# clysto/tinyimgcodec

Hardware: AMD Instinct MI355X
Metric: Mpixels/s encode (DCT+quant kernel) (higher is better)
Workload: dtype f32+f64

## Files before the change

### tinyimgcodec_amd/csrc/tic_kernels.hip

```cpp
#include <hip/hip_runtime.h>
#include <hip/hip_ext.h>
#include <stdint.h>
#include <stdlib.h>
#include <string.h>
#include <type_traits>

#include "tic_hooks.h"
#include "tic_kernels.h"
#include "tic_math.h"

namespace tic {

#define TIC_DPP_QP_XOR1 0xB1
#define TIC_DPP_QP_XOR2 0x4E
#define TIC_DPP_ROW_SHL4 0x104
#define TIC_DPP_ROW_SHR4 0x114

__device__ __forceinline__ uint32_t perm_b32(uint32_t hi_src, uint32_t lo_src, uint32_t sel) {
    return __builtin_amdgcn_perm(hi_src, lo_src, sel);
}

__device__ __forceinline__ void transpose8x8_bytes(uint32_t &lo, uint32_t &hi, int i) {
    uint32_t nhi = (uint32_t)__builtin_amdgcn_update_dpp((int)hi, (int)lo, TIC_DPP_ROW_SHL4, 0xf, 0x5, false);
    uint32_t nlo = (uint32_t)__builtin_amdgcn_update_dpp((int)lo, (int)hi, TIC_DPP_ROW_SHR4, 0xf, 0xa, false);
    lo = nlo;
    hi = nhi;
    uint32_t selB = (i & 2) ? 0x03020706u : 0x05040100u;
    uint32_t plo = (uint32_t)__builtin_amdgcn_mov_dpp((int)lo, TIC_DPP_QP_XOR2, 0xf, 0xf, true);
    uint32_t phi = (uint32_t)__builtin_amdgcn_mov_dpp((int)hi, TIC_DPP_QP_XOR2, 0xf, 0xf, true);
    lo = perm_b32(plo, lo, selB);
    hi = perm_b32(phi, hi, selB);
    uint32_t selC = (i & 1) ? 0x03070105u : 0x06020400u;
    plo = (uint32_t)__builtin_amdgcn_mov_dpp((int)lo, TIC_DPP_QP_XOR1, 0xf, 0xf, true);
    phi = (uint32_t)__builtin_amdgcn_mov_dpp((int)hi, TIC_DPP_QP_XOR1, 0xf, 0xf, true);
    lo = perm_b32(plo, lo, selC);
    hi = perm_b32(phi, hi, selC);
}

__device__ __forceinline__ void transpose8x8_bytes_shfl(uint32_t &lo, uint32_t &hi, int i) {
    uint32_t row[2] = {lo, hi};
    uint32_t col_lo = 0, col_hi = 0;
    int base = (threadIdx.x & 63) & ~7;
    for (int r = 0; r < 8; r++) {
        uint32_t l = __shfl(row[0], base + r, 64), h = __shfl(row[1], base + r, 64);
        uint32_t w = (i < 4) ? l : h;
        uint32_t byte = (w >> (8 * (i & 3))) & 0xffu;
        if (r < 4)
            col_lo |= byte << (8 * r);
        else
            col_hi |= byte << (8 * (r - 4));
    }
    lo = col_lo;
    hi = col_hi;
}

__device__ __forceinline__ void wave_lds_fence() {
    __builtin_amdgcn_fence(__ATOMIC_RELEASE, "wavefront");
    __builtin_amdgcn_wave_barrier();
    __builtin_amdgcn_fence(__ATOMIC_ACQUIRE, "wavefront");
}

__device__ __forceinline__ int reflect_index(int i, int n) {
    if (i < n) return i;
    if (n >= 8) return 2 * (n - 1) - i;
    if (n == 1) return 0;
    int p = 2 * (n - 1), j = i;
    while (j >= p) j -= p;
    return j < n ? j : p - j;
}

constexpr int kWavesPerWG = 4;
constexpr int kLdsStrideDw = 68;
constexpr int kZzStrideB = 144;
constexpr int kLdsWaveBytes = 8 * kLdsStrideDw * 4;

struct Strip {
    int by, bx;
    bool valid;
    size_t oblk;
};

__device__ __forceinline__ void load_block_row(const uint8_t *__restrict__ img, int h, int w, long stride, bool aligned8,
                                               const Strip &s, int i, uint32_t &lo, uint32_t &hi) {
    lo = 0;
    hi = 0;
    if (!s.valid) return;
    int y = reflect_index(s.by * 8 + i, h);
    int x0 = s.bx * 8;
    const uint8_t *p = img + (long)y * stride + x0;
    if (aligned8 && x0 + 8 <= w) {
        uint2 v = *reinterpret_cast<const uint2 *>(p);
        lo = v.x;
        hi = v.y;
    } else {
        const uint8_t *rowp = img + (long)y * stride;
#pragma unroll
        for (int k = 0; k < 8; k++) {
            uint32_t b = rowp[reflect_index(x0 + k, w)];
            if (k < 4)
                lo |= b << (8 * k);
            else
                hi |= b << (8 * (k - 4));
        }
    }
}

__device__ __forceinline__ void transpose8x8_dwords(uint32_t *lds, int b, int i, uint32_t v[8]) {
    uint32_t *blk = lds + b * kLdsStrideDw;
#pragma unroll
    for (int u = 0; u < 8; u++) blk[u * 8 + i] = v[u];
    wave_lds_fence();
    const uint4 *rp = reinterpret_cast<const uint4 *>(blk + i * 8);
    uint4 a = rp[0], c = rp[1];
    v[0] = a.x; v[1] = a.y; v[2] = a.z; v[3] = a.w;
    v[4] = c.x; v[5] = c.y; v[6] = c.z; v[7] = c.w;
    wave_lds_fence();
}

__device__ __forceinline__ void exact_block(uint32_t colLo, uint32_t colHi, uint32_t *lds, int b, int i,
                                         const DctqConsts *__restrict__ C, int q[8]) {
    double c[8];
#pragma unroll
    for (int r = 0; r < 4; r++) {
        c[r] = (double)((int)((colLo >> (8 * r)) & 0xffu) - 128);
        c[r + 4] = (double)((int)((colHi >> (8 * r)) & 0xffu) - 128);
    }
    dct8_exact(c[0], c[1], c[2], c[3], c[4], c[5], c[6], c[7]);
    uint32_t w[8];
#pragma unroll
    for (int k = 0; k < 8; k++) w[k] = (uint32_t)__double2loint(c[k]);
    transpose8x8_dwords(lds, b, i, w);
    uint32_t wh[8];
#pragma unroll
    for (int k = 0; k < 8; k++) wh[k] = (uint32_t)__double2hiint(c[k]);
    transpose8x8_dwords(lds, b, i, wh);
#pragma unroll
    for (int k = 0; k < 8; k++) c[k] = __hiloint2double((int)wh[k], (int)w[k]);
    dct8_exact(c[0], c[1], c[2], c[3], c[4], c[5], c[6], c[7]);
    const double *div = C->div + i * 8;
#pragma unroll
    for (int v = 0; v < 8; v++) {
        q[v] = (int)rint(c[v] / div[v]);
        __builtin_amdgcn_sched_barrier(0);
    }
}

__device__ __forceinline__ void store_zigzag(uint32_t *lds, int b, int i, const uint16_t zz[8], const int q[8],
                                             int16_t *__restrict__ out, const Strip &s) {
    char *blk = reinterpret_cast<char *>(lds) + b * kZzStrideB;
#pragma unroll
    for (int v = 0; v < 8; v++) *reinterpret_cast<int16_t *>(blk + zz[v]) = (int16_t)q[v];
    wave_lds_fence();
    uint4 val = *reinterpret_cast<const uint4 *>(blk + i * 16);
    wave_lds_fence();
    if (s.valid) *reinterpret_cast<uint4 *>(out + s.oblk * 64 + i * 8) = val;
}

__device__ __forceinline__ Strip make_strip(int tile, int ntiles, int tiles_x, int bw, int b) {
    Strip s;
    int ty = tile / tiles_x;
    int tx = tile - ty * tiles_x;
    s.by = ty;
    s.bx = tx * 8 + b;
    s.valid = (tile < ntiles) && (s.bx < bw);
    s.oblk = (size_t)ty * bw + s.bx;
    return s;
}

__global__ __launch_bounds__(kWavesPerWG * 64) void dctq_exact_kernel(DctqArgs a) {
    __shared__ __attribute__((aligned(16))) uint32_t lds_all[kWavesPerWG][kLdsWaveBytes / 4];
    a.img += (long)blockIdx.y * a.frame_stride_in;
    a.out = reinterpret_cast<int16_t *>(reinterpret_cast<char *>(a.out) + (long)blockIdx.y * a.frame_stride_out);
    const int lane = threadIdx.x & 63, wave = threadIdx.x >> 6;
    const int b = lane >> 3, i = lane & 7;
    uint32_t *lds = lds_all[wave];
    int tile = blockIdx.x * kWavesPerWG + wave;
    int ntiles = a.ntiles;
    if (a.rem_mode) {
        const int bh = a.ntiles / a.tiles_x, rw = a.tiles_x - a.fast_tx;
        const int n_right = bh * rw, n_bottom = (bh - a.fast_ty) * a.fast_tx;
        ntiles = 0;
        if (tile < n_right) {
            tile = (tile / rw) * a.tiles_x + a.fast_tx + tile % rw;
            ntiles = a.ntiles;
        } else if (tile < n_right + n_bottom) {
            const int k = tile - n_right;
            tile = (a.fast_ty + k / a.fast_tx) * a.tiles_x + k % a.fast_tx;
            ntiles = a.ntiles;
        }
    }
    Strip s = make_strip(tile, ntiles, a.tiles_x, a.bw, b);
    uint32_t lo, hi;
    load_block_row(a.img, a.h, a.w, a.stride, a.aligned8, s, i, lo, hi);
    transpose8x8_bytes(lo, hi, i);
    int q[8];
    exact_block(lo, hi, lds, b, i, a.consts, q);
    const uint4 zzv = *reinterpret_cast<const uint4 *>(a.consts->zzofs + i * 8);
    uint16_t zz[8] = {(uint16_t)zzv.x, (uint16_t)(zzv.x >> 16), (uint16_t)zzv.y, (uint16_t)(zzv.y >> 16),
                      (uint16_t)zzv.z, (uint16_t)(zzv.z >> 16), (uint16_t)zzv.w, (uint16_t)(zzv.w >> 16)};
    store_zigzag(lds, b, i, zz, q, a.out, s);
}

constexpr int kTWaveBytes = kLdsWaveBytes;
constexpr int kTHalfDw = 272;
constexpr int kZzWaveBytes = 8 * kZzStrideB;
constexpr int kPxBlkBytes = 80;
constexpr int kMaxStripsPerWave = 16;
constexpr int kChunkStrips = 8;

__device__ __forceinline__ void quant_fma(float z, float mul, uint32_t &bits, float &d) {
    const float s = fmaf(z, mul, kMagic);
    bits = __float_as_uint(s);
    const float nr = kMagic - s;
    d = fmaf(z, mul, nr);
}

__device__ __forceinline__ void store16_wt_nt(void *p, const uint4 &v) {
    typedef uint32_t u32x4 __attribute__((ext_vector_type(4)));
    const u32x4 d = {v.x, v.y, v.z, v.w};
    asm volatile("global_store_dwordx4 %0, %1, off sc1 nt" : : "v"(p), "v"(d) : "memory");
}
__device__ __forceinline__ void store16_wt_nt(const void *sbase, uint32_t voff, const uint4 &v) {
    typedef uint32_t u32x4 __attribute__((ext_vector_type(4)));
    const u32x4 d = {v.x, v.y, v.z, v.w};
    asm volatile("global_store_dwordx4 %0, %1, %2 sc1 nt" : : "v"(voff), "v"(d), "s"(sbase) : "memory");
}

constexpr int kMaxStripsPerWave2 = 64;
constexpr int kBatch = 8;
constexpr int kBatchWaveBytes = kBatch * (128 + 64) + 64;

template <int CTRL>
__device__ __forceinline__ double dpp_f64(double x) {
    const int lo = __builtin_amdgcn_mov_dpp(__double2loint(x), CTRL, 0xf, 0xf, true);
    const int hi = __builtin_amdgcn_mov_dpp(__double2hiint(x), CTRL, 0xf, 0xf, true);
    return __hiloint2double(hi, lo);
}

__device__ __forceinline__ int rational_quad(const uint32_t *ldsT, int b, int i, const double *cst_rat) {
#pragma clang fp contract(off)
    const int w = i >> 2, k = i & 3;
    const uint32_t ca = (0x05010300u >> (8 * k)) & 0xffu, cb = (0x06020407u >> (8 * k)) & 0xffu;
    const uint32_t *row = ldsT + w * 128 + 4 * b;
    const float fa = __uint_as_float(row[(ca >> 2) * kTHalfDw + (ca & 3)]);
    const float fb = __uint_as_float(row[(cb >> 2) * kTHalfDw + (cb & 3)]);
    const double K = w ? (kTW3 * 0.5) : (kSq2h * 0.5);
    const double ya = (double)fa * K, yb = (double)fb * K;
    const double p = ya + yb;
    const double s2 = p + dpp_f64<TIC_DPP_QP_XOR1>(p);
    const double o = dpp_f64<TIC_DPP_QP_XOR2>(s2);
    const double E = (k & 1) ? s2 - o : s2 + o;
    const double X = E * ((k & 1) ? (kTW3 * 0.5) : (kSq2h * 0.5));
    const double div = cst_rat[2 * w + (k & 1)], rdiv = cst_rat[4 + 2 * w + (k & 1)];
    return (int)rint(div_rn(X, div, rdiv));
}

__device__ __forceinline__ int rational_slim(uint32_t rowLo, uint32_t rowHi, int i, const double *cst_rat) {
#pragma clang fp contract(off)
    uint32_t lo = perm_b32(rowHi, rowLo, 0x04030700u);
    uint32_t hi = perm_b32(rowHi, rowLo, 0x06050201u);
    transpose8x8_bytes(lo, hi, i);
    const uint32_t tot = __builtin_amdgcn_sad_u8(lo, 0u, __builtin_amdgcn_sad_u8(hi, 0u, 0u));
    const uint32_t sa = __builtin_amdgcn_sad_u8(lo & 0xff0000ffu, 0u, __builtin_amdgcn_sad_u8(hi & 0xff0000ffu, 0u, 0u));
    const int e0 = (int)tot - 1024, e4 = 2 * (int)sa - (int)tot;
    double y0 = (double)e0 * (kSq2h * 0.5);
    double y4 = (double)e4 * (kTW3 * 0.5);
    y0 = y0 + dpp_f64<TIC_DPP_QP_XOR1>(y0);
    y4 = y4 + dpp_f64<TIC_DPP_QP_XOR1>(y4);
    y0 = y0 + dpp_f64<TIC_DPP_QP_XOR2>(y0);
    y4 = y4 + dpp_f64<TIC_DPP_QP_XOR2>(y4);
    const double b0 = dpp_f64<TIC_DPP_ROW_SHL4>(y0), b4 = dpp_f64<TIC_DPP_ROW_SHL4>(y4);
    const double A = (i & 2) ? y4 : y0, B = (i & 2) ? b4 : b0;
    const double E = (i & 1) ? A - B : A + B;
    const double X = E * ((i & 1) ? (kTW3 * 0.5) : (kSq2h * 0.5));
    const double div = cst_rat[i & 3], rdiv = cst_rat[4 + (i & 3)];
    return (int)rint(div_rn(X, div, rdiv));
}
__device__ __forceinline__ unsigned long long wave_redo_block(const uint8_t *px , double *tbuf ,
                                                              const double *cosm, const double *rdiv, const uint16_t *zzofs, int16_t *img16,
                                                              int lane) {
    const int u = lane >> 3, c = lane & 7;
    typedef double d2 __attribute__((ext_vector_type(2)));
    const d2 *mu = reinterpret_cast<const d2 *>(cosm + u * 8), *mc = reinterpret_cast<const d2 *>(cosm + c * 8);
    const d2 m0 = mu[0], m1 = mu[1], m2 = mu[2], m3 = mu[3];
    double x[8];
#pragma unroll
    for (int r = 0; r < 8; r++) x[r] = (double)((int)px[r * 8 + c] - 128);
    double ta = m0.x * x[0], tb = m0.y * x[1];
    ta = fma(m1.x, x[2], ta); tb = fma(m1.y, x[3], tb);
    ta = fma(m2.x, x[4], ta); tb = fma(m2.y, x[5], tb);
    ta = fma(m3.x, x[6], ta); tb = fma(m3.y, x[7], tb);
    tbuf[u * 8 + c] = ta + tb;
    const d2 n0 = mc[0], n1 = mc[1], n2 = mc[2], n3 = mc[3];
    wave_lds_fence();
    const d2 *tu = reinterpret_cast<const d2 *>(tbuf + u * 8);
    const d2 y0 = tu[0], y1 = tu[1], y2 = tu[2], y3 = tu[3];
    double xa = n0.x * y0.x, xb = n0.y * y0.y;
    xa = fma(n1.x, y1.x, xa); xb = fma(n1.y, y1.y, xb);
    xa = fma(n2.x, y2.x, xa); xb = fma(n2.y, y2.y, xb);
    xa = fma(n3.x, y3.x, xa); xb = fma(n3.y, y3.y, xb);
    const double X = xa + xb;
    const double tq = X * rdiv[lane], rq = rint(tq);
    const bool rational = (lane & 0x1b) == 0;
    const bool decided = fabs(tq - rq) < 0.5 - 1e-9;
    if (decided && !rational) img16[zzofs[lane] >> 1] = (int16_t)(int)rq;
    const unsigned long long und = __ballot(!decided && !rational);
    wave_lds_fence();
    return und;
}

__device__ __forceinline__ uint32_t second_level_8(uint32_t colLo, uint32_t colHi, uint32_t *lds, int b, int i, const double *mul64, int q[8]) {
    double c[8];
#pragma unroll
    for (int r = 0; r < 4; r++) {
        c[r] = (double)(int)((colLo >> (8 * r)) & 0xffu);
        c[r + 4] = (double)(int)((colHi >> (8 * r)) & 0xffu);
    }
    dct8_aan(c[0], c[1], c[2], c[3], c[4], c[5], c[6], c[7]);
    c[0] -= 1024.0;
    uint32_t w[8], wh[8];
#pragma unroll
    for (int k = 0; k < 8; k++) w[k] = (uint32_t)__double2loint(c[k]);
    transpose8x8_dwords(lds, b, i, w);
#pragma unroll
    for (int k = 0; k < 8; k++) wh[k] = (uint32_t)__double2hiint(c[k]);
    transpose8x8_dwords(lds, b, i, wh);
#pragma unroll
    for (int k = 0; k < 8; k++) c[k] = __hiloint2double((int)wh[k], (int)w[k]);
    dct8_aan(c[0], c[1], c[2], c[3], c[4], c[5], c[6], c[7]);
    uint32_t und = 0;
#pragma unroll
    for (int v = 0; v < 8; v++) {
        const double t = c[v] * mul64[i * 8 + v], r = rint(t);
        q[v] = (int)r;
        if (!(fabs(t - r) < 0.5 - 1e-9)) und |= 1u << v;
    }
    return und;
}

template <bool kCols>
__global__ __launch_bounds__(kWavesPerWG * 64, 6) __attribute__((amdgpu_num_vgpr(72))) void dctq_strip_kernel(DctqArgs a) {
    __shared__ __attribute__((aligned(16))) uint32_t ldsT_all[kWavesPerWG][kTWaveBytes / 4];
    __shared__ __attribute__((aligned(16))) uint32_t ldsZ_all[kWavesPerWG][kZzWaveBytes / 4];
    __shared__ __attribute__((aligned(16))) unsigned char cst_blk[kStripBlkBytes];
    __shared__ __attribute__((aligned(16))) uint32_t bat_all[kWavesPerWG][kBatchWaveBytes / 4];
    const int lane = threadIdx.x & 63;
    const int wave = __builtin_amdgcn_readfirstlane(threadIdx.x >> 6);
    uint32_t *ldsT = ldsT_all[wave];
    char *ldsZ = reinterpret_cast<char *>(ldsZ_all[wave]);
    const uint16_t *cst_zz = reinterpret_cast<const uint16_t *>(cst_blk + kBlkZz);
    const double *cst_rat = reinterpret_cast<const double *>(cst_blk + kBlkRat);
    uint4 *bat_img = reinterpret_cast<uint4 *>(bat_all[wave]);
    uint2 *bat_pix = reinterpret_cast<uint2 *>(bat_all[wave] + kBatch * 32);
    uint32_t *bat_id = bat_all[wave] + kBatch * 48;
    const DctqConsts *__restrict__ C = a.consts;
    a.img += (long)blockIdx.z * a.frame_stride_in;
    a.out = reinterpret_cast<int16_t *>(reinterpret_cast<char *>(a.out) + (long)blockIdx.z * a.frame_stride_out);

    const int lr = lane >> 3, lb = lane & 7;
    const int b = lane >> 3, i = lane & 7;
    unsigned long long mask_exact = 0;
    uint32_t n_second = 0, n_quad = 0;
    int nE = 0;
    int t_first, n_my;
    const uint32_t st_off = (uint32_t)lane * 16u;
    {
        typedef float f32x4 __attribute__((ext_vector_type(4)));
        typedef uint32_t u32x4 __attribute__((ext_vector_type(4)));
        f32x4 m0, m1;
        f32x4 thr;
        u32x4 zzv;
        u32x4 c_fill;
        {
            constexpr int kPpw = kStripBlkPieces / kWavesPerWG;
            static_assert(kPpw * kWavesPerWG == kStripBlkPieces && kPpw <= 64, "constant block must split evenly over the waves");
            const uint32_t piece = lane < kPpw ? (uint32_t)(wave * kPpw + lane) : (uint32_t)kStripBlkPieces - 1u;
            const uint32_t fo = piece * 16u;
            asm volatile("global_load_dwordx4 v[76:79], %0, %1" : : "v"(fo), "s"(C->strip_blk) : "memory", "v76", "v77", "v78", "v79");
        }
        const uint32_t px_wr = (uint32_t)(uintptr_t)(__attribute__((address_space(3))) char *)(ldsZ + lb * kPxBlkBytes + lr * 8);
        const uint8_t *px_rd = reinterpret_cast<const uint8_t *>(ldsZ + b * kPxBlkBytes + i);
        constexpr int kHalf = kCols ? kTHalfDw : 256;
        const int p1a = kCols ? i : lr, p1b = kCols ? b : lb;
        uint32_t *twA = ldsT + (p1a >> 2) * kHalf + (p1a & 3) + 4 * p1b;
        uint32_t *twB = ldsT + (p1a >> 2) * kHalf + (p1a & 3) + 4 * (p1b ^ 4);
        const uint4 *tr = reinterpret_cast<const uint4 *>(
            __builtin_assume_aligned(ldsT + i * 32 + 4 * (b ^ (4 * ((i >> 1) & 1))), 16));
        const uint32_t ld_off = (uint32_t)(lr * (int)a.stride + lb * 8);

        uint32_t tf, t_lim;
        if (a.team_count > 0) {
            const uint32_t r = blockIdx.y;
            const uint32_t row0 = (uint32_t)((r < 8u ? a.split_lo >> (8u * r) : a.split_hi) & 0xffull);
            const uint32_t row1 = (uint32_t)((r < 7u ? a.split_lo >> (8u * r + 8u) : a.split_hi) & 0xffull);
            tf = (row0 * (uint32_t)a.team_count + blockIdx.x) * kWavesPerWG + (uint32_t)wave;
            t_lim = tf + (row1 - row0) * (uint32_t)a.tstep;
        } else if (a.round_wgs > 0) {
            const uint32_t rho = a.magic_tstep ? __umulhi(blockIdx.x, a.magic_tstep ) : blockIdx.x;
            const uint32_t wl = blockIdx.x - rho * (uint32_t)a.round_wgs;
            const uint32_t base = rho * (uint32_t)a.round_wgs * (uint32_t)a.wg_span;
            tf = base + wl * kWavesPerWG + (uint32_t)wave;
            t_lim = base + (uint32_t)a.round_wgs * (uint32_t)a.wg_span;
        } else {
            tf = blockIdx.x * (uint32_t)a.wg_stride + (uint32_t)wave;
            t_lim = blockIdx.x * (uint32_t)a.wg_stride + (uint32_t)a.wg_span;
        }
        tf = __builtin_amdgcn_readfirstlane(tf);
        const uint32_t nfast = (uint32_t)a.fast_ty * (uint32_t)a.fast_tx;
        const uint32_t t_end = t_lim < nfast ? t_lim : nfast;
        n_my = 0;
        if (tf < t_end) n_my = (a.round_wgs > 0 || a.magic_tstep == 0u) ? (int)((t_end - tf + (uint32_t)a.tstep - 1u) / (uint32_t)a.tstep)
                                                                        : (int)__umulhi(t_end - tf + (uint32_t)a.tstep - 1u, a.magic_tstep);
        if (n_my == 0) tf = 0;
        t_first = (int)tf;
        const uint32_t ty_first = a.magic_fast_tx ? __umulhi(tf, a.magic_fast_tx) : tf;
        int txp = (int)(tf - ty_first * (uint32_t)a.fast_tx);
        uint32_t in_off = ty_first * (uint32_t)(8 * a.stride) + (uint32_t)txp * 64u;
        uint32_t oblk = ty_first * (uint32_t)a.bw + (uint32_t)txp * 8u;
        uint32_t src_off = 0;
        int n_issued = 0;
        const uint8_t *img_s = a.img;
#define TIC_RSV_CLOBBER "memory", "v72", "v73", "v74", "v75", "v76", "v77", "v78", "v79"
#define TIC_LOAD(R, OB)                                                                                      \
    do {                                                                                                     \
        src_off = n_issued < n_my ? in_off : src_off;                                                        \
        OB = oblk;                                                                                           \
        asm volatile("global_load_dwordx2 v[" R "], %0, %1" : : "v"(ld_off), "s"(img_s + src_off) : TIC_RSV_CLOBBER); \
        n_issued++; txp += a.step_tx; in_off += a.in_step32; oblk += a.oblk_step;                            \
        if (__builtin_expect(txp >= a.fast_tx, 0)) { txp -= a.fast_tx; in_off += a.in_wrap32; oblk += a.oblk_wrap; } \
    } while (0)
#define TIC_TAKE_COLS(R, N) asm volatile("s_waitcnt vmcnt(" #N ")\n\tds_write_b64 %0, v[" R "]" : : "v"(px_wr) : TIC_RSV_CLOBBER)
#define TIC_TAKE_ROWS(D, R0, R1, N)                                                                          \
    asm volatile("s_waitcnt vmcnt(" #N ")\n\tv_cvt_f32_ubyte0 %0, v" #R0 "\n\tv_cvt_f32_ubyte1 %1, v" #R0 "\n\tv_cvt_f32_ubyte2 %2, v" #R0 \
                 "\n\tv_cvt_f32_ubyte3 %3, v" #R0 "\n\tv_cvt_f32_ubyte0 %4, v" #R1 "\n\tv_cvt_f32_ubyte1 %5, v" #R1                       \
                 "\n\tv_cvt_f32_ubyte2 %6, v" #R1 "\n\tv_cvt_f32_ubyte3 %7, v" #R1                                                       \
                 : "=v"(D[0]), "=v"(D[1]), "=v"(D[2]), "=v"(D[3]), "=v"(D[4]), "=v"(D[5]), "=v"(D[6]), "=v"(D[7]) : : TIC_RSV_CLOBBER)
        uint32_t ob0, ob1, ob2;
        uint32_t kstrip = 0;
        TIC_LOAD("72:73", ob0);
        TIC_LOAD("74:75", ob1);
        asm volatile("s_waitcnt vmcnt(2)\n\tv_mov_b32 %0, v76\n\tv_mov_b32 %1, v77\n\tv_mov_b32 %2, v78\n\tv_mov_b32 %3, v79"
                     : "=v"(c_fill.x), "=v"(c_fill.y), "=v"(c_fill.z), "=v"(c_fill.w) : : "memory", "v76", "v77", "v78", "v79");
        if (lane < kStripBlkPieces / kWavesPerWG) *reinterpret_cast<u32x4 *>(cst_blk + (wave * (kStripBlkPieces / kWavesPerWG) + lane) * 16) = c_fill;
        asm volatile("s_waitcnt lgkmcnt(0)\n\ts_barrier" : : : "memory");
        m0 = *reinterpret_cast<const f32x4 *>(cst_blk + (kCols ? kBlkMul : kBlkMulT) + i * 32);
        m1 = *reinterpret_cast<const f32x4 *>(cst_blk + (kCols ? kBlkMul : kBlkMulT) + i * 32 + 16);
        thr = *reinterpret_cast<const f32x4 *>(cst_blk + (kCols ? kBlkThr : kBlkThrT) + i * 16);
        zzv = *reinterpret_cast<const u32x4 *>(cst_blk + (kCols ? kBlkZz : kBlkZzT) + i * 16);
        auto zz_ptr = [&](uint32_t ofs) {
            const uint32_t c = ofs >> 4;
            return reinterpret_cast<int16_t *>(ldsZ + c * 128 + (ofs & 15) + 16 * (b ^ (kCols ? (((c >> 1) & 1) | (c & 4)) : (4 * ((c >> 1) & 1)))));
        };
        int16_t *zp0 = zz_ptr(zzv.x & 0xffff), *zp1 = zz_ptr(zzv.x >> 16), *zp2 = zz_ptr(zzv.y & 0xffff), *zp3 = zz_ptr(zzv.y >> 16);
        int16_t *zp4 = zz_ptr(zzv.z & 0xffff), *zp5 = zz_ptr(zzv.z >> 16), *zp6 = zz_ptr(zzv.w & 0xffff), *zp7 = zz_ptr(zzv.w >> 16);
        const uint4 *zr = reinterpret_cast<const uint4 *>(
            __builtin_assume_aligned(ldsZ + 16 * (i * 8 + (b ^ (kCols ? (((i >> 1) & 1) | (i & 4)) : (4 * ((i >> 1) & 1))))), 16));
        wave_lds_fence();

        int left = n_my;
        auto raw_words = [&](auto tag, uint32_t &lo, uint32_t &hi) {
            constexpr int R = decltype(tag)::value;
            static_assert(R == 72 || R == 74 || R == 76, "landing register pair");
            if constexpr (R == 72) asm volatile("v_mov_b32 %0, v72\n\tv_mov_b32 %1, v73" : "=v"(lo), "=v"(hi) : : "memory");
            else if constexpr (R == 74) asm volatile("v_mov_b32 %0, v74\n\tv_mov_b32 %1, v75" : "=v"(lo), "=v"(hi) : : "memory");
            else asm volatile("v_mov_b32 %0, v76\n\tv_mov_b32 %1, v77" : "=v"(lo), "=v"(hi) : : "memory");
        };
        auto process = [&](auto tag, const float (&pxr)[8], const uint32_t ob) {
            float d0, d1, d2, d3, d4, d5, d6, d7;
            if constexpr (kCols) {
                d0 = (float)px_rd[0]; d1 = (float)px_rd[8]; d2 = (float)px_rd[16]; d3 = (float)px_rd[24];
                d4 = (float)px_rd[32]; d5 = (float)px_rd[40]; d6 = (float)px_rd[48]; d7 = (float)px_rd[56];
            } else {
                d0 = pxr[0]; d1 = pxr[1]; d2 = pxr[2]; d3 = pxr[3]; d4 = pxr[4]; d5 = pxr[5]; d6 = pxr[6]; d7 = pxr[7];
            }
            dct8_aan(d0, d1, d2, d3, d4, d5, d6, d7);
            d0 -= 1024.0f;
            twA[0 * 32] = __float_as_uint(d0); twA[1 * 32] = __float_as_uint(d1); twB[2 * 32] = __float_as_uint(d2);
            twB[3 * 32] = __float_as_uint(d3); twA[4 * 32] = __float_as_uint(d4); twA[5 * 32] = __float_as_uint(d5);
            twB[6 * 32] = __float_as_uint(d6); twB[7 * 32] = __float_as_uint(d7);
            wave_lds_fence();
            const uint4 ra = tr[0], rb = tr[kHalf / 4];
            wave_lds_fence();
            float e0 = __uint_as_float(ra.x), e1 = __uint_as_float(ra.y), e2 = __uint_as_float(ra.z), e3 = __uint_as_float(ra.w);
            float e4 = __uint_as_float(rb.x), e5 = __uint_as_float(rb.y), e6 = __uint_as_float(rb.z), e7 = __uint_as_float(rb.w);
            dct8_aan(e0, e1, e2, e3, e4, e5, e6, e7);
            uint32_t q0, q1, q2, q3, q4, q5, q6, q7;
            float r0, r1, r2, r3, r4, r5, r6, r7;
            quant_fma(e0, m0.x, q0, r0); quant_fma(e1, m0.y, q1, r1); quant_fma(e2, m0.z, q2, r2); quant_fma(e3, m0.w, q3, r3);
            quant_fma(e4, m1.x, q4, r4); quant_fma(e5, m1.y, q5, r5); quant_fma(e6, m1.z, q6, r6); quant_fma(e7, m1.w, q7, r7);
            const float mA1 = fmaxf(fmaxf(fabsf(r1), fabsf(r2)), fabsf(r3));
            const float mA2 = fmaxf(fmaxf(fabsf(r5), fabsf(r6)), fabsf(r7));
            const float mB = fmaxf(fabsf(r0), fabsf(r4));
            const unsigned long long cA = __ballot(mA1 > thr.x) | __ballot(mA2 > thr.y);
            const unsigned long long cB = __ballot(mB > thr.z);
            *zp0 = (int16_t)q0; *zp1 = (int16_t)q1; *zp2 = (int16_t)q2; *zp3 = (int16_t)q3;
            *zp4 = (int16_t)q4; *zp5 = (int16_t)q5; *zp6 = (int16_t)q6; *zp7 = (int16_t)q7;
            const unsigned long long kRat = 0x1111111111111111ull;
            if (__builtin_expect((cB & kRat) != 0ull, 0)) {
                n_quad++;
                if constexpr (kCols) {
                    const int rq = rational_quad(ldsT, b, i, cst_rat);
                    if ((i & 2) == 0) *zz_ptr(28u * (uint32_t)(i & 1) + 20u * (uint32_t)(i >> 2) + 30u * (uint32_t)((i & 1) & (i >> 2))) = (int16_t)rq;
                } else {
                    uint32_t lo0, hi0;
                    raw_words(tag, lo0, hi0);
                    uint2 *pb = reinterpret_cast<uint2 *>(ldsT);
                    pb[lb * 8 + lr] = make_uint2(lo0, hi0);
                    wave_lds_fence();
                    const uint2 rowv = pb[lane];
                    wave_lds_fence();
                    const int rq = rational_slim(rowv.x, rowv.y, i, cst_rat);
                    if (i < 4) *zz_ptr(i == 0 ? 0u : (i == 1 ? 28u : (i == 2 ? 20u : 78u))) = (int16_t)rq;
                }
            }
            wave_lds_fence();
            const uint4 val = *zr;
            wave_lds_fence();
            const char *dst = reinterpret_cast<const char *>(a.out) + ((unsigned long long)ob << 7);
            const unsigned long long mG = cA | (cB & ~kRat);
            if (__builtin_expect(mG != 0ull, 0)) {
                const uint32_t gm = (uint32_t)__ballot(((mG >> (8u * (uint32_t)i)) & 0xffull) != 0ull) & 0xffu;
                const int nnew = __builtin_popcount(gm);
                if (nE + nnew <= kBatch && gm != 0xffu) {
                    uint32_t lo0, hi0;
                    raw_words(tag, lo0, hi0);
                    const uint32_t below = (1u << b) - 1u, lbelow = (1u << lb) - 1u;
                    const bool mine = (gm >> b) & 1u;
                    const int e = nE + __builtin_popcount(gm & below);
                    if (mine) bat_img[e * 8 + i] = val;
                    if (mine && i == 0) bat_id[e] = ob + (uint32_t)b;
                    if ((gm >> lb) & 1u) bat_pix[(nE + __builtin_popcount(gm & lbelow)) * 8 + lr] = make_uint2(lo0, hi0);
                    if (!mine) store16_wt_nt(dst, st_off, val);
                    nE += nnew;
                    n_second += (uint32_t)nnew;
                } else {
                    mask_exact |= 1ull << kstrip;
                    store16_wt_nt(dst, st_off, val);
                }
            } else
                store16_wt_nt(dst, st_off, val);
            left--;
            kstrip++;
        };
        float pxf[8] = {0.f, 0.f, 0.f, 0.f, 0.f, 0.f, 0.f, 0.f};
#define TIC_STEP(RLOAD, OBL, RTAKE, R0, R1, OBP, N)                                                          \
        TIC_LOAD(RLOAD, OBL);                                                                                \
        if constexpr (kCols) { TIC_TAKE_COLS(RTAKE, N); } else { TIC_TAKE_ROWS(pxf, R0, R1, N); }            \
        process(std::integral_constant<int, R0>(), pxf, OBP)
        do {
            if (left == 0) break;
            TIC_STEP("76:77", ob2, "72:73", 72, 73, ob0, 2);
            if (left == 0) break;
            TIC_STEP("72:73", ob0, "74:75", 74, 75, ob1, 3);
            while (left != 0) {
                TIC_STEP("74:75", ob1, "76:77", 76, 77, ob2, 4);
                if (left == 0) break;
                TIC_STEP("76:77", ob2, "72:73", 72, 73, ob0, 4);
                if (left == 0) break;
                TIC_STEP("72:73", ob0, "74:75", 74, 75, ob1, 4);
            }
        } while (0);
#undef TIC_STEP
        asm volatile("; end of the strip walk" : : : TIC_RSV_CLOBBER);
#undef TIC_LOAD
#undef TIC_TAKE_COLS
#undef TIC_TAKE_ROWS
#undef TIC_RSV_CLOBBER
    }
    if (nE != 0) {
        const double *cst_cos = reinterpret_cast<const double *>(cst_blk + kBlkCos);
        const double *cst_rdiv = reinterpret_cast<const double *>(cst_blk + kBlkRdiv);
        uint32_t m_exact = 0;
        if (nE < 3) {
            for (int ee = 0; ee < nE; ee++) {
                const unsigned long long und = wave_redo_block(reinterpret_cast<const uint8_t *>(bat_pix + ee * 8), reinterpret_cast<double *>(ldsT), cst_cos,
                                                               cst_rdiv, cst_zz, reinterpret_cast<int16_t *>(bat_img + ee * 8), lane);
                if (und != 0ull) m_exact |= 1u << ee;
            }
        } else {
            const bool have2 = b < nE;
            const int e2 = have2 ? b : 0;
            const uint2 rowv = bat_pix[e2 * 8 + i];
            uint32_t lo = rowv.x, hi = rowv.y;
            transpose8x8_bytes(lo, hi, i);
            int qs[8];
            uint32_t und = second_level_8(lo, hi, ldsT, b, i, reinterpret_cast<const double *>(cst_blk + kBlkMul64), qs);
            if ((i & 3) == 0) und &= ~0x11u;
            const uint4 zo = *reinterpret_cast<const uint4 *>(cst_zz + i * 8);
            const uint32_t zw[4] = {zo.x, zo.y, zo.z, zo.w};
            int16_t *img2 = reinterpret_cast<int16_t *>(bat_img + e2 * 8);
            if (have2) {
#pragma unroll
                for (int v = 0; v < 8; v++)
                    if (!((und >> v) & 1u) && !((i & 3) == 0 && (v & 3) == 0)) img2[((zw[v >> 1] >> (16 * (v & 1))) & 0xffffu) >> 1] = (int16_t)qs[v];
            }
            const unsigned long long um = __ballot(have2 && und != 0u);
            for (int ee = 0; ee < nE; ee++)
                if ((um >> (8 * ee)) & 0xffull) m_exact |= 1u << ee;
        }
        const bool have = b < nE;
        const int e = have ? b : 0;
        const uint32_t blk = bat_id[e];
        if (m_exact != 0u) {
            const uint2 rowv = bat_pix[e * 8 + i];
            int16_t *img16 = reinterpret_cast<int16_t *>(bat_img + e * 8);
            uint32_t lo = rowv.x, hi = rowv.y;
            transpose8x8_bytes(lo, hi, i);
            const uint4 zo = *reinterpret_cast<const uint4 *>(cst_zz + i * 8);
            const uint32_t zw[4] = {zo.x, zo.y, zo.z, zo.w};
            int qx[8];
            exact_block(lo, hi, ldsT, b, i, C, qx);
            if (have && ((m_exact >> e) & 1u)) {
#pragma unroll
                for (int v = 0; v < 8; v++) img16[((zw[v >> 1] >> (16 * (v & 1))) & 0xffffu) >> 1] = (int16_t)qx[v];
            }
        }
        wave_lds_fence();
        const uint4 val = bat_img[e * 8 + i];
        if (have) store16_wt_nt(reinterpret_cast<char *>(a.out) + ((unsigned long long)blk << 7) + (uint32_t)i * 16u, val);
    }
    if (a.fallback_count != nullptr && lane == 0) {
        if (n_second != 0) atomicAdd(a.fallback_count, (unsigned long long)n_second);
        if (n_quad != 0) atomicAdd(a.fallback_count + 1, (unsigned long long)n_quad);
        if (mask_exact != 0ull) atomicAdd(a.fallback_count + 2, (unsigned long long)__builtin_popcountll(mask_exact));
        if (nE != 0) atomicMax(a.fallback_count + 3, (unsigned long long)nE);
    }
    if (mask_exact == 0ull) return;
    asm volatile("s_waitcnt vmcnt(0)" : : : "memory");
    const uint4 zzn = *reinterpret_cast<const uint4 *>(cst_zz + i * 8);
    const uint16_t zz[8] = {(uint16_t)zzn.x, (uint16_t)(zzn.x >> 16), (uint16_t)zzn.y, (uint16_t)(zzn.y >> 16),
                            (uint16_t)zzn.z, (uint16_t)(zzn.z >> 16), (uint16_t)zzn.w, (uint16_t)(zzn.w >> 16)};
    for (unsigned long long todo = mask_exact; todo != 0ull; todo &= todo - 1ull) {
        const int k = __builtin_ctzll(todo);
        const long t = (long)t_first + (long)k * a.tstep;
        const int ty = (int)(t / a.fast_tx), tx = (int)(t - (long)ty * a.fast_tx);
        Strip s;
        s.by = ty;
        s.bx = tx * 8 + b;
        s.valid = true;
        s.oblk = (size_t)ty * a.bw + s.bx;
        uint32_t lo, hi;
        load_block_row(a.img, a.h, a.w, a.stride, true, s, i, lo, hi);
        transpose8x8_bytes(lo, hi, i);
        int q[8];
        const uint32_t und = second_level_8(lo, hi, ldsT, b, i, reinterpret_cast<const double *>(cst_blk + kBlkMul64), q);
        if (__ballot(und != 0u) != 0ull) exact_block(lo, hi, ldsT, b, i, C, q);
        store_zigzag(reinterpret_cast<uint32_t *>(ldsZ), b, i, zz, q, a.out, s);
    }
}

__global__ __launch_bounds__(kWavesPerWG * 64) void dctq_exact_wide_kernel(WideArgs a) {
    __shared__ __attribute__((aligned(16))) uint32_t lds_all[kWavesPerWG][kLdsWaveBytes / 4];
    const int lane = threadIdx.x & 63, wave = threadIdx.x >> 6;
    const int b = lane >> 3, i = lane & 7;
    uint32_t *lds = lds_all[wave];
    const int tile = blockIdx.x * kWavesPerWG + wave;
    Strip s = make_strip(tile, a.ntiles, a.tiles_x, a.bw, b);
    double c[8];
#pragma unroll
    for (int r = 0; r < 8; r++) c[r] = 0.0;
    if (s.valid) {
        const int x = reflect_index(s.bx * 8 + i, a.w);
#pragma unroll
        for (int r = 0; r < 8; r++) {
            const int y = reflect_index(s.by * 8 + r, a.h);
            c[r] = (double)a.img[(long)y * a.stride + x] - 128.0;
        }
    }
    dct8_exact(c[0], c[1], c[2], c[3], c[4], c[5], c[6], c[7]);
    uint32_t w[8], wh[8];
#pragma unroll
    for (int k = 0; k < 8; k++) w[k] = (uint32_t)__double2loint(c[k]);
    transpose8x8_dwords(lds, b, i, w);
#pragma unroll
    for (int k = 0; k < 8; k++) wh[k] = (uint32_t)__double2hiint(c[k]);
    transpose8x8_dwords(lds, b, i, wh);
#pragma unroll
    for (int k = 0; k < 8; k++) c[k] = __hiloint2double((int)wh[k], (int)w[k]);
    dct8_exact(c[0], c[1], c[2], c[3], c[4], c[5], c[6], c[7]);
    if (!s.valid) return;
    const double *div = a.consts->div + i * 8;
    const uint16_t *zz = a.consts->zzofs + i * 8;
    int32_t *ob = a.out + s.oblk * 64;
#pragma unroll
    for (int v = 0; v < 8; v++) {
        ob[zz[v] >> 1] = (int32_t)rint(c[v] / div[v]);
        __builtin_amdgcn_sched_barrier(0);
    }
}

__constant__ int kAnnScalesInt[64] = {
    16384, 22725, 21407, 19266, 16384, 12873, 8867,  4520,  22725, 31521, 29692, 26722, 22725, 17855, 12299, 6270,
    21407, 29692, 27969, 25172, 21407, 16819, 11585, 5906,  19266, 26722, 25172, 22654, 19266, 15137, 10426, 5315,
    16384, 22725, 21407, 19266, 16384, 12873, 8867,  4520,  12873, 17855, 16819, 15137, 12873, 10114, 6967,  3552,
    8867,  12299, 11585, 10426, 8867,  6967,  4799,  2446,  4520,  6270,  5906,  5315,  4520,  3552,  2446,  1247};

template <bool kWideDc, bool kMeasure = false>
__device__ __forceinline__ void idct_body(const IdctArgs &a, int wg_tile0, const SseArgs *m = nullptr) {
    __shared__ __attribute__((aligned(16))) uint32_t lds_all[kWavesPerWG][kLdsWaveBytes / 4];
    const int lane = threadIdx.x & 63, wave = threadIdx.x >> 6;
    const int b = lane >> 3, i = lane & 7;
    uint32_t *lds = lds_all[wave];
    const int tile = wg_tile0 + wave;
    const DctqConsts *__restrict__ C = a.consts;
    Strip s = make_strip(tile, a.ntiles, a.tiles_x, a.bw, b);
    if (a.first_block >= 0) {
        const long blk = a.first_block + (long)tile * 8 + b;
        s.valid = blk < a.first_block + a.nblocks_sel;
        s.by = (int)(blk / a.bw);
        s.bx = (int)(blk - (long)s.by * a.bw);
        s.oblk = (size_t)blk;
    }

    uint4 val = make_uint4(0, 0, 0, 0);
    if (s.valid) val = *reinterpret_cast<const uint4 *>(a.coeffs + s.oblk * 64 + i * 8);
    char *blk = reinterpret_cast<char *>(lds) + b * kZzStrideB;
    {
        uint32_t wv[4] = {val.x, val.y, val.z, val.w};
#pragma unroll
        for (int k = 0; k < 8; k++) {
            int nat = C->zznat[i * 8 + k];
            int16_t cv = (int16_t)((wv[k >> 1] >> (16 * (k & 1))) & 0xffffu);
            *reinterpret_cast<int16_t *>(blk + nat * 2) = cv;
        }
    }
    wave_lds_fence();
    double c[8];
#pragma unroll
    for (int u = 0; u < 8; u++) {
        int16_t cv = *reinterpret_cast<const int16_t *>(blk + (u * 8 + i) * 2);
        if (a.scaled)
            c[u] = (((double)cv / ((double)kAnnScalesInt[u * 8 + i] / 2048.0)) * a.pow2) * C->div[u * 8 + i];
        else
            c[u] = (double)cv * C->div[u * 8 + i];
    }
    if (kWideDc && i == 0 && s.valid) {
        const double dcv = (double)a.dc32[s.oblk];
        c[0] = a.scaled ? ((dcv / ((double)kAnnScalesInt[0] / 2048.0)) * a.pow2) * C->div[0] : dcv * C->div[0];
    }
    wave_lds_fence();
    idct8_exact(c[0], c[1], c[2], c[3], c[4], c[5], c[6], c[7]);
    uint32_t w[8], wh[8];
#pragma unroll
    for (int k = 0; k < 8; k++) w[k] = (uint32_t)__double2loint(c[k]);
    transpose8x8_dwords(lds, b, i, w);
#pragma unroll
    for (int k = 0; k < 8; k++) wh[k] = (uint32_t)__double2hiint(c[k]);
    transpose8x8_dwords(lds, b, i, wh);
#pragma unroll
    for (int k = 0; k < 8; k++) c[k] = __hiloint2double((int)wh[k], (int)w[k]);
    idct8_exact(c[0], c[1], c[2], c[3], c[4], c[5], c[6], c[7]);
    uint32_t px[8];
#pragma unroll
    for (int k = 0; k < 8; k++) {
        double v = c[k] + 128.0;
        v = v < 0.0 ? 0.0 : v;
        v = v > 255.0 ? 255.0 : v;
        px[k] = (uint32_t)(int)v;
    }
    if constexpr (kMeasure) {
        __shared__ uint32_t wsum[kWavesPerWG][2];
        uint32_t sq = 0, sw = 0;
        const int y = s.by * 8 + i, x0 = s.bx * 8;
        if (s.valid && y < a.h) {
            const uint8_t *p = m->img + (long)y * m->stride + x0;
            uint32_t lo = 0, hi = 0;
            if (m->aligned8 && x0 + 8 <= a.w) {
                const uint2 v = *reinterpret_cast<const uint2 *>(p);
                lo = v.x;
                hi = v.y;
            } else {
#pragma unroll
                for (int k = 0; k < 8; k++)
                    if (x0 + k < a.w) {
                        const uint32_t bt = p[k];
                        if (k < 4) lo |= bt << (8 * k); else hi |= bt << (8 * (k - 4));
                    }
            }
#pragma unroll
            for (int k = 0; k < 8; k++) {
                const int d = (int)px[k] - (int)(((k < 4 ? lo : hi) >> (8 * (k & 3))) & 0xffu);
                const uint32_t e = x0 + k < a.w ? (uint32_t)(d * d) : 0u;
                sq += e;
                sw += e & 255u;
            }
        }
#pragma unroll
        for (int off = 32; off > 0; off >>= 1) {
            sq += (uint32_t)__shfl_xor((int)sq, off, 64);
            sw += (uint32_t)__shfl_xor((int)sw, off, 64);
        }
        if (lane == 0) {
            wsum[wave][0] = sq;
            wsum[wave][1] = sw;
        }
        __syncthreads();
        if (threadIdx.x == 0) {
            unsigned long long tq = 0, tw = 0;
#pragma unroll
            for (int k = 0; k < kWavesPerWG; k++) {
                tq += wsum[k][0];
                tw += wsum[k][1];
            }
            if (tq) atomicAdd(&m->res->sse, tq);
            if (tw) atomicAdd(&m->res->sse_wrapped, tw);
        }
        return;
    }
    if (!s.valid) return;
    int y = s.by * 8 + i;
    if (y >= a.h) return;
    int x0 = s.bx * 8;
    uint8_t *p = a.out + (long)y * a.stride + x0;
    if (a.aligned8 && x0 + 8 <= a.w) {
        uint2 o;
        o.x = px[0] | (px[1] << 8) | (px[2] << 16) | (px[3] << 24);
        o.y = px[4] | (px[5] << 8) | (px[6] << 16) | (px[7] << 24);
        *reinterpret_cast<uint2 *>(p) = o;
    } else {
#pragma unroll
        for (int k = 0; k < 8; k++)
            if (x0 + k < a.w) p[k] = (uint8_t)px[k];
    }
}
__global__ __launch_bounds__(kWavesPerWG * 64) void idct_kernel(IdctArgs a) { idct_body<false>(a, blockIdx.x * kWavesPerWG); }
__global__ __launch_bounds__(kWavesPerWG * 64) void idct_wide_dc_kernel(IdctArgs a) { idct_body<true>(a, blockIdx.x * kWavesPerWG); }
__global__ __launch_bounds__(kWavesPerWG * 64) void idct_sse_kernel(IdctArgs a, SseArgs m) { idct_body<false, true>(a, blockIdx.x * kWavesPerWG, &m); }
__global__ __launch_bounds__(kWavesPerWG * 64) void idct_batch_kernel(const IdctArgs *__restrict__ args, const uint2 *__restrict__ wgs) {
    const uint2 e = wgs[blockIdx.x];
    const IdctArgs a = args[e.x];
    idct_body<false>(a, (int)e.y);
}

__global__ void selftest_transpose_kernel(const uint2 *in, uint2 *out_dpp, uint2 *out_ref) {
    int lane = threadIdx.x & 63, i = lane & 7;
    uint2 v = in[blockIdx.x * blockDim.x + threadIdx.x];
    uint32_t lo = v.x, hi = v.y;
    transpose8x8_bytes(lo, hi, i);
    out_dpp[blockIdx.x * blockDim.x + threadIdx.x] = make_uint2(lo, hi);
    lo = v.x;
    hi = v.y;
    transpose8x8_bytes_shfl(lo, hi, i);
    out_ref[blockIdx.x * blockDim.x + threadIdx.x] = make_uint2(lo, hi);
}

static inline int grid_for(int ntiles) { return (ntiles + kWavesPerWG - 1) / kWavesPerWG; }

struct Tunables {
    int max_wgs, sched, chunk, order;
    int split[8];
};
static Tunables read_tunables() {
    auto geti = [](const char *k, int d) { const char *v = test_hook(k); return v ? atoi(v) : d; };
    Tunables t;
    t.max_wgs = geti("TIC_MAX_WGS", 0);
    t.sched = geti("TIC_SCHED", 1);
    t.chunk = geti("TIC_CHUNK", kChunkStrips);
    t.order = geti("TIC_ORDER", -1);
    const char *sp = test_hook("TIC_SPLIT") ? test_hook("TIC_SPLIT") : "15,13,10,7,5,3";
    for (int k = 0; k < 8; k++) t.split[k] = 0;
    for (int k = 0; k < 8 && sp && *sp; k++) {
        t.split[k] = atoi(sp);
        sp = strchr(sp, ',');
        if (sp) sp++;
    }
    return t;
}
static Tunables tunables() {
    static const bool live = test_hook("TIC_TUNE") != nullptr;
    static const Tunables once = read_tunables();
    return live ? read_tunables() : once;
}

int dctq_kernel_id(int abi_variant) {
    return abi_variant == 1 ? 1 : ((abi_variant == 0 || abi_variant == 2) ? 2 : -1);
}

hipError_t launch_dctq(DctqArgs a, int variant, hipStream_t stream, hipEvent_t ev_start, hipEvent_t ev_stop) {
    if (a.ntiles <= 0) return hipSuccess;
    if (variant != 1 && variant != 2) return hipErrorInvalidValue;
    dim3 block(kWavesPerWG * 64);
    a.nwaves = a.step_ty = a.step_tx = 0;
    a.fast_ty = a.fast_tx = 0;
    a.rem_mode = 0;
    a.dbg = nullptr;
    const int nf = a.nframes > 0 ? a.nframes : 1;
    if (variant == 1) {
        hipLaunchKernelGGL(dctq_exact_kernel, dim3(grid_for(a.ntiles), nf), block, 0, stream, a);
        return hipGetLastError();
    }
    {
        long limit = 1L << 32;
        if (const char *e = test_hook("TIC_BAND_BYTES")) limit = atol(e) > 0 ? atol(e) : limit;
        if (a.aligned8 && nf == 1 && a.w >= 64 && (long)a.h * a.stride >= limit) {
            const long band = (limit - 1) / a.stride / 8 * 8;
            if (band >= 8) {
                for (long y0 = 0; y0 < a.h; y0 += band) {
                    DctqArgs b = a;
                    b.h = (int)((long)a.h - y0 < band ? (long)a.h - y0 : band);
                    b.img = a.img + y0 * a.stride;
                    b.out = a.out + (y0 / 8) * (long)a.bw * 64;
                    b.ntiles = ((b.h + 7) / 8) * b.tiles_x;
                    const hipError_t e = launch_dctq(b, variant, stream);
                    if (e != hipSuccess) return e;
                }
                return hipSuccess;
            }
        }
    }
    const int bh = a.ntiles / a.tiles_x;
    a.fast_tx = (a.aligned8 && (long)a.h * a.stride < (1L << 32)) ? a.w / 64 : 0;
    a.fast_ty = a.h / 8;
    const int nfast = a.fast_tx * a.fast_ty;
    if (nfast > 0) {
        const int max_strips = kMaxStripsPerWave2;
        int wgs = grid_for(nfast);
        static int cus = 256;
        static const int resident = [] {
            int dev = 0, per_cu = 0;
            hipDeviceProp_t prop;
            if (hipGetDevice(&dev) == hipSuccess && hipGetDeviceProperties(&prop, dev) == hipSuccess) cus = prop.multiProcessorCount;
            if (hipOccupancyMaxActiveBlocksPerMultiprocessor(&per_cu, dctq_strip_kernel<true>, kWavesPerWG * 64, 0) != hipSuccess || per_cu < 1)
                per_cu = 4;
            if (per_cu > 6) per_cu = 6;
            return cus * per_cu;
        }();
        const Tunables tune = tunables();
        const int cap_env = tune.max_wgs > 0 ? tune.max_wgs : resident;
        int cap = cap_env / nf;
        if (cap < 64) cap = 64;
        if (wgs > cap) wgs = cap;
        const int min_wgs = (nfast + kWavesPerWG * max_strips - 1) / (kWavesPerWG * max_strips);
        if (wgs < min_wgs) wgs = min_wgs;
        a.nwaves = wgs * kWavesPerWG;
        a.wg_stride = kWavesPerWG;
        a.tstep = a.nwaves;
        a.wg_span = nfast;
        a.round_wgs = 0;
        a.team_count = 0;
        const int S = tune.chunk < 1 ? 1 : (tune.chunk > max_strips ? max_strips : tune.chunk);
        const int min_wgs16 = (nfast + kWavesPerWG * kMaxStripsPerWave - 1) / (kWavesPerWG * kMaxStripsPerWave);
        const bool multi_round = (long)min_wgs16 * nf > (long)cap_env;
        if (tune.sched == 1 && multi_round) {
            a.wg_stride = a.wg_span = kWavesPerWG * S;
            a.tstep = kWavesPerWG;
            wgs = (nfast + a.wg_stride - 1) / a.wg_stride;
            a.nwaves = wgs * kWavesPerWG;
        } else if (tune.sched == 2 && multi_round && nf == 1) {
            a.round_wgs = cap_env;
            a.wg_span = kWavesPerWG * S;
            a.tstep = a.round_wgs * kWavesPerWG;
            wgs = (nfast + a.wg_span - 1) / a.wg_span;
            wgs = (wgs + a.round_wgs - 1) / a.round_wgs * a.round_wgs;
            a.nwaves = wgs * kWavesPerWG;
        }
        if (!multi_round && nf == 1 && tune.split[0] > 0 && wgs == cap_env && wgs % cus == 0 && wgs / cus <= 8) {
            const int R = wgs / cus;
            a.team_count = cus;
            a.tstep = cus * kWavesPerWG;
            const int rows_total = (nfast + a.tstep - 1) / a.tstep;
            double wsum = 0;
            for (int r = 0; r < R; r++) wsum += tune.split[r] > 0 ? tune.split[r] : 1;
            double acc = 0;
            a.split[0] = 0;
            for (int r = 0; r < R; r++) {
                acc += tune.split[r] > 0 ? tune.split[r] : 1;
                a.split[r + 1] = (int)(rows_total * acc / wsum + 0.5);
                if (a.split[r + 1] - a.split[r] > max_strips) a.team_count = 0;
            }
            a.split[R] = rows_total;
            if (rows_total > 255) a.team_count = 0;
            if (a.team_count == 0) a.tstep = a.nwaves;
        }
        a.step_ty = a.tstep / a.fast_tx;
        a.step_tx = a.tstep % a.fast_tx;
        a.in_step32 = (uint32_t)((long)a.step_ty * 8 * a.stride + (long)a.step_tx * 64);
        a.in_wrap32 = (uint32_t)(8 * a.stride - (long)a.fast_tx * 64);
        a.oblk_step = (uint32_t)((long)a.step_ty * a.bw + (long)a.step_tx * 8);
        a.oblk_wrap = (uint32_t)((long)a.bw - (long)a.fast_tx * 8);
        dim3 grid(wgs, 1, nf);
        const unsigned long long dmax = (unsigned long long)(a.round_wgs > 0 ? a.round_wgs : a.tstep);
        if ((unsigned long long)nfast * (unsigned long long)a.fast_tx >= (1ull << 32) ||
            ((unsigned long long)nfast + dmax) * dmax >= (1ull << 32)) {
            a.fast_tx = a.fast_ty = 0;
        } else {
            auto magic = [](long d) { return d <= 1 ? 0u : (uint32_t)((1ull << 32) / (unsigned long long)d + 1ull); };
            a.magic_fast_tx = magic(a.fast_tx);
            a.magic_tstep = magic(a.round_wgs > 0 ? a.round_wgs : a.tstep);
            a.split_lo = a.split_hi = 0;
            if (a.team_count > 0) {
                const int R = wgs / a.team_count;
                for (int k = 0; k <= R; k++) {
                    if (k < 8) a.split_lo |= (unsigned long long)(a.split[k] & 0xff) << (8 * k);
                    else a.split_hi = (unsigned long long)(a.split[k] & 0xff);
                }
                grid = dim3(a.team_count, R, nf);
            }
            const bool cols = tune.order < 0 ? !multi_round : tune.order == 1;
            if (ev_start && ev_stop) {
                if (cols)
                    hipExtLaunchKernelGGL(dctq_strip_kernel<true>, grid, block, 0, stream, ev_start, ev_stop, 0, a);
                else
                    hipExtLaunchKernelGGL(dctq_strip_kernel<false>, grid, block, 0, stream, ev_start, ev_stop, 0, a);
            } else if (cols)
                hipLaunchKernelGGL(dctq_strip_kernel<true>, grid, block, 0, stream, a);
            else
                hipLaunchKernelGGL(dctq_strip_kernel<false>, grid, block, 0, stream, a);
        }
    } else {
        a.fast_tx = a.fast_ty = 0;
    }
    const int nrem = bh * (a.tiles_x - a.fast_tx) + (bh - a.fast_ty) * a.fast_tx;
    if (nrem > 0) {
        a.rem_mode = 1;
        hipLaunchKernelGGL(dctq_exact_kernel, dim3(grid_for(nrem), nf), block, 0, stream, a);
    }
    return hipGetLastError();
}

hipError_t launch_dctq_wide(const WideArgs &a, hipStream_t stream) {
    if (a.ntiles <= 0) return hipSuccess;
    hipLaunchKernelGGL(dctq_exact_wide_kernel, dim3(grid_for(a.ntiles)), dim3(kWavesPerWG * 64), 0, stream, a);
    return hipGetLastError();
}

hipError_t launch_idct(const IdctArgs &a, hipStream_t stream) {
    if (a.ntiles <= 0) return hipSuccess;
    dim3 grid(grid_for(a.ntiles)), block(kWavesPerWG * 64);
    if (a.dc32) hipLaunchKernelGGL(idct_wide_dc_kernel, grid, block, 0, stream, a);
    else hipLaunchKernelGGL(idct_kernel, grid, block, 0, stream, a);
    return hipGetLastError();
}

int idct_batch_wgs(int ntiles) { return grid_for(ntiles); }
int idct_batch_tiles_per_wg() { return kWavesPerWG; }
hipError_t launch_idct_batch(const IdctArgs *d_args, const uint2 *d_wgs, size_t nwgs, hipStream_t stream) {
    if (!d_args || !d_wgs || nwgs == 0 || nwgs > 0x7fffffffu) return hipErrorInvalidValue;
    hipLaunchKernelGGL(idct_batch_kernel, dim3((uint32_t)nwgs), dim3(kWavesPerWG * 64), 0, stream, d_args, d_wgs);
    return hipGetLastError();
}

hipError_t launch_idct_sse(const IdctArgs &a, const SseArgs &m, hipStream_t stream) {
    if (a.ntiles <= 0) return hipSuccess;
    hipLaunchKernelGGL(idct_sse_kernel, dim3(grid_for(a.ntiles)), dim3(kWavesPerWG * 64), 0, stream, a, m);
    return hipGetLastError();
}

hipError_t launch_selftest_transpose(const void *in, void *out_dpp, void *out_ref, int nthreads, hipStream_t stream) {
    hipLaunchKernelGGL(selftest_transpose_kernel, dim3(nthreads / 256), dim3(256), 0, stream, (const uint2 *)in,
                       (uint2 *)out_dpp, (uint2 *)out_ref);
    return hipGetLastError();
}

}
```

Before: 1.733 million.

## Pack strip-kernel kernargs into hot scalar head and one warm line

Moves the strip-schedule planning into a shared header and passes the kernel a compact set of leading scalar arguments plus a 64-byte warm struct, keeping the full DctqArgs only for the rare fallback paths. The prologue computes the cursor from these fewer scalars and issues the first image loads before computing output block indices and LDS addresses. The goal is to shorten the kernel prologue by cutting scalar kernarg loads and address arithmetic ahead of the first global loads. It adds a larger kernarg block and inline-asm register pinning that depend on the compiler honouring the new layout.

Result: faster. 1.766 million (median of 6 runs) (+1.9%).

```diff
diff --git a/tinyimgcodec_amd/csrc/tic_kernels.hip b/tinyimgcodec_amd/csrc/tic_kernels.hip
--- a/tinyimgcodec_amd/csrc/tic_kernels.hip
+++ b/tinyimgcodec_amd/csrc/tic_kernels.hip
@@ -1,5 +1,6 @@
 #include <hip/hip_runtime.h>
 #include <hip/hip_ext.h>
+#include <stddef.h>
 #include <stdint.h>
 #include <stdlib.h>
 #include <string.h>
@@ -7,6 +8,7 @@
 
 #include "tic_hooks.h"
 #include "tic_kernels.h"
+#include "tic_strip_plan.h"
 #include "tic_math.h"
 
 namespace tic {
@@ -70,6 +72,7 @@
 }
 
 constexpr int kWavesPerWG = 4;
+static_assert(kWavesPerWG == kStripWavesPerWG, "tic_strip_plan.h plans for this workgroup");
 constexpr int kLdsStrideDw = 68;
 constexpr int kZzStrideB = 144;
 constexpr int kLdsWaveBytes = 8 * kLdsStrideDw * 4;
@@ -205,7 +208,6 @@
 constexpr int kTHalfDw = 272;
 constexpr int kZzWaveBytes = 8 * kZzStrideB;
 constexpr int kPxBlkBytes = 80;
-constexpr int kMaxStripsPerWave = 16;
 constexpr int kChunkStrips = 8;
 
 __device__ __forceinline__ void quant_fma(float z, float mul, uint32_t &bits, float &d) {
@@ -226,7 +228,6 @@
     asm volatile("global_store_dwordx4 %0, %1, %2 sc1 nt" : : "v"(voff), "v"(d), "s"(sbase) : "memory");
 }
 
-constexpr int kMaxStripsPerWave2 = 64;
 constexpr int kBatch = 8;
 constexpr int kBatchWaveBytes = kBatch * (128 + 64) + 64;
 
@@ -338,8 +339,29 @@
     return und;
 }
 
+struct StripKernargs {
+    const uint8_t *img;
+    const DctqConsts *consts;
+    StripHead hd;
+    StripWarm w;
+    DctqArgs a;
+};
+static_assert(offsetof(StripKernargs, hd) == 16 && sizeof(StripHead) == 40 && offsetof(StripKernargs, w) == 64, "leading scalars, then one line");
+
+template <class T>
+__device__ __forceinline__ uint32_t lds_addr(T *p) {
+    return (uint32_t)(uintptr_t)(__attribute__((address_space(3))) char *)(p);
+}
+template <class T>
+__device__ __forceinline__ T *lds_ptr(uint32_t v) {
+    return (T *)(__attribute__((address_space(3))) T *)(uintptr_t)v;
+}
+
 template <bool kCols>
-__global__ __launch_bounds__(kWavesPerWG * 64, 6) __attribute__((amdgpu_num_vgpr(72))) void dctq_strip_kernel(DctqArgs a) {
+__global__ __launch_bounds__(kWavesPerWG * 64, 6) __attribute__((amdgpu_num_vgpr(72))) void dctq_strip_kernel(
+    const uint8_t *img, const DctqConsts *consts, unsigned long long hd_split, uint32_t hd_stride, uint32_t hd_misc, uint32_t hd_tstep,
+    uint32_t hd_nfast, uint32_t hd_fast_tx, uint32_t hd_magic_fast_tx, uint32_t hd_in_step32, uint32_t hd_step_tx, StripWarm w, DctqArgs a) {
+    const StripHead hd = {hd_split, hd_stride, hd_misc, hd_tstep, hd_nfast, hd_fast_tx, hd_magic_fast_tx, hd_in_step32, hd_step_tx};
     __shared__ __attribute__((aligned(16))) uint32_t ldsT_all[kWavesPerWG][kTWaveBytes / 4];
     __shared__ __attribute__((aligned(16))) uint32_t ldsZ_all[kWavesPerWG][kZzWaveBytes / 4];
     __shared__ __attribute__((aligned(16))) unsigned char cst_blk[kStripBlkBytes];
@@ -353,9 +375,12 @@
     uint4 *bat_img = reinterpret_cast<uint4 *>(bat_all[wave]);
     uint2 *bat_pix = reinterpret_cast<uint2 *>(bat_all[wave] + kBatch * 32);
     uint32_t *bat_id = bat_all[wave] + kBatch * 48;
-    const DctqConsts *__restrict__ C = a.consts;
-    a.img += (long)blockIdx.z * a.frame_stride_in;
-    a.out = reinterpret_cast<int16_t *>(reinterpret_cast<char *>(a.out) + (long)blockIdx.z * a.frame_stride_out);
+    const DctqConsts *__restrict__ C = consts;
+    const uint8_t *img_s = img;
+    if (__builtin_expect(blockIdx.z != 0, 0)) {
+        asm volatile("" : : : "memory");
+        img_s += (long)blockIdx.z * w.frame_stride_in;
+    }
 
     const int lr = lane >> 3, lb = lane & 7;
     const int b = lane >> 3, i = lane & 7;
@@ -363,7 +388,8 @@
     uint32_t n_second = 0, n_quad = 0;
     int nE = 0;
     int t_first, n_my;
-    const uint32_t st_off = (uint32_t)lane * 16u;
+    int16_t *out_f;
+    uint32_t st_off = (uint32_t)lane * 16u;
     {
         typedef float f32x4 __attribute__((ext_vector_type(4)));
         typedef uint32_t u32x4 __attribute__((ext_vector_type(4)));
@@ -378,56 +404,30 @@
             const uint32_t fo = piece * 16u;
             asm volatile("global_load_dwordx4 v[76:79], %0, %1" : : "v"(fo), "s"(C->strip_blk) : "memory", "v76", "v77", "v78", "v79");
         }
-        const uint32_t px_wr = (uint32_t)(uintptr_t)(__attribute__((address_space(3))) char *)(ldsZ + lb * kPxBlkBytes + lr * 8);
-        const uint8_t *px_rd = reinterpret_cast<const uint8_t *>(ldsZ + b * kPxBlkBytes + i);
-        constexpr int kHalf = kCols ? kTHalfDw : 256;
-        const int p1a = kCols ? i : lr, p1b = kCols ? b : lb;
-        uint32_t *twA = ldsT + (p1a >> 2) * kHalf + (p1a & 3) + 4 * p1b;
-        uint32_t *twB = ldsT + (p1a >> 2) * kHalf + (p1a & 3) + 4 * (p1b ^ 4);
-        const uint4 *tr = reinterpret_cast<const uint4 *>(
-            __builtin_assume_aligned(ldsT + i * 32 + 4 * (b ^ (4 * ((i >> 1) & 1))), 16));
-        const uint32_t ld_off = (uint32_t)(lr * (int)a.stride + lb * 8);
-
-        uint32_t tf, t_lim;
-        if (a.team_count > 0) {
-            const uint32_t r = blockIdx.y;
-            const uint32_t row0 = (uint32_t)((r < 8u ? a.split_lo >> (8u * r) : a.split_hi) & 0xffull);
-            const uint32_t row1 = (uint32_t)((r < 7u ? a.split_lo >> (8u * r + 8u) : a.split_hi) & 0xffull);
-            tf = (row0 * (uint32_t)a.team_count + blockIdx.x) * kWavesPerWG + (uint32_t)wave;
-            t_lim = tf + (row1 - row0) * (uint32_t)a.tstep;
-        } else if (a.round_wgs > 0) {
-            const uint32_t rho = a.magic_tstep ? __umulhi(blockIdx.x, a.magic_tstep ) : blockIdx.x;
-            const uint32_t wl = blockIdx.x - rho * (uint32_t)a.round_wgs;
-            const uint32_t base = rho * (uint32_t)a.round_wgs * (uint32_t)a.wg_span;
-            tf = base + wl * kWavesPerWG + (uint32_t)wave;
-            t_lim = base + (uint32_t)a.round_wgs * (uint32_t)a.wg_span;
-        } else {
-            tf = blockIdx.x * (uint32_t)a.wg_stride + (uint32_t)wave;
-            t_lim = blockIdx.x * (uint32_t)a.wg_stride + (uint32_t)a.wg_span;
-        }
-        tf = __builtin_amdgcn_readfirstlane(tf);
-        const uint32_t nfast = (uint32_t)a.fast_ty * (uint32_t)a.fast_tx;
-        const uint32_t t_end = t_lim < nfast ? t_lim : nfast;
-        n_my = 0;
-        if (tf < t_end) n_my = (a.round_wgs > 0 || a.magic_tstep == 0u) ? (int)((t_end - tf + (uint32_t)a.tstep - 1u) / (uint32_t)a.tstep)
-                                                                        : (int)__umulhi(t_end - tf + (uint32_t)a.tstep - 1u, a.magic_tstep);
-        if (n_my == 0) tf = 0;
-        t_first = (int)tf;
-        const uint32_t ty_first = a.magic_fast_tx ? __umulhi(tf, a.magic_fast_tx) : tf;
-        int txp = (int)(tf - ty_first * (uint32_t)a.fast_tx);
-        uint32_t in_off = ty_first * (uint32_t)(8 * a.stride) + (uint32_t)txp * 64u;
-        uint32_t oblk = ty_first * (uint32_t)a.bw + (uint32_t)txp * 8u;
+        const uint32_t ld_off = (uint32_t)lr * hd.stride + (uint32_t)lb * 8u;
+
+        const StripCursor cur = strip_cursor(hd, w, blockIdx.x, blockIdx.y, (uint32_t)wave);
+        n_my = cur.n_my;
+        t_first = (int)cur.t_first;
+        uint32_t txp = cur.txp, in_off = cur.in_off, oblk;
+        const uint32_t in_wrap32 = strip_in_wrap(hd);
         uint32_t src_off = 0;
         int n_issued = 0;
-        const uint8_t *img_s = a.img;
 #define TIC_RSV_CLOBBER "memory", "v72", "v73", "v74", "v75", "v76", "v77", "v78", "v79"
 #define TIC_LOAD(R, OB)                                                                                      \
     do {                                                                                                     \
         src_off = n_issued < n_my ? in_off : src_off;                                                        \
         OB = oblk;                                                                                           \
         asm volatile("global_load_dwordx2 v[" R "], %0, %1" : : "v"(ld_off), "s"(img_s + src_off) : TIC_RSV_CLOBBER); \
-        n_issued++; txp += a.step_tx; in_off += a.in_step32; oblk += a.oblk_step;                            \
-        if (__builtin_expect(txp >= a.fast_tx, 0)) { txp -= a.fast_tx; in_off += a.in_wrap32; oblk += a.oblk_wrap; } \
+        n_issued++;                                                                                          \
+        strip_step(txp, in_off, oblk, hd.step_tx, hd.fast_tx, hd.in_step32, in_wrap32, w);                   \
+    } while (0)
+#define TIC_LOAD_HEAD(R, WRAP)                                                                               \
+    do {                                                                                                     \
+        src_off = n_issued < n_my ? in_off : src_off;                                                        \
+        asm volatile("global_load_dwordx2 v[" R "], %0, %1" : : "v"(ld_off), "s"(img_s + src_off) : TIC_RSV_CLOBBER); \
+        n_issued++;                                                                                          \
+        WRAP = strip_step_in(txp, in_off, hd.step_tx, hd.fast_tx, hd.in_step32, in_wrap32);                  \
     } while (0)
 #define TIC_TAKE_COLS(R, N) asm volatile("s_waitcnt vmcnt(" #N ")\n\tds_write_b64 %0, v[" R "]" : : "v"(px_wr) : TIC_RSV_CLOBBER)
 #define TIC_TAKE_ROWS(D, R0, R1, N)                                                                          \
@@ -437,8 +437,32 @@
                  : "=v"(D[0]), "=v"(D[1]), "=v"(D[2]), "=v"(D[3]), "=v"(D[4]), "=v"(D[5]), "=v"(D[6]), "=v"(D[7]) : : TIC_RSV_CLOBBER)
         uint32_t ob0, ob1, ob2;
         uint32_t kstrip = 0;
-        TIC_LOAD("72:73", ob0);
-        TIC_LOAD("74:75", ob1);
+        bool wrap0, wrap1;
+        uint32_t ty0 = cur.ty, tx0 = cur.txp;
+        TIC_LOAD_HEAD("72:73", wrap0);
+        TIC_LOAD_HEAD("74:75", wrap1);
+        asm volatile("; block indices: behind the loads" : "+s"(ty0), "+s"(tx0) : "s"(w.round_wgs), "s"(w.round_span), "s"(w.magic_round_wgs) : TIC_RSV_CLOBBER);
+        oblk = strip_oblk(ty0, tx0, w);
+        ob0 = oblk;
+        strip_step_blk(oblk, wrap0, w);
+        ob1 = oblk;
+        strip_step_blk(oblk, wrap1, w);
+        constexpr int kHalf = kCols ? kTHalfDw : 256;
+        const int p1a = kCols ? i : lr, p1b = kCols ? b : lb;
+        uint32_t px_wr = lds_addr(ldsZ + lb * kPxBlkBytes + lr * 8);
+        uint32_t o_px_rd = lds_addr(ldsZ + b * kPxBlkBytes + i);
+        uint32_t o_twA = lds_addr(ldsT + (p1a >> 2) * kHalf + (p1a & 3) + 4 * p1b);
+        uint32_t o_twB = lds_addr(ldsT + (p1a >> 2) * kHalf + (p1a & 3) + 4 * (p1b ^ 4));
+        uint32_t q_tr = (uint32_t)(i * 8 + (b ^ (4 * ((i >> 1) & 1))));
+        uint32_t q_zr = (uint32_t)(i * 8 + (b ^ (kCols ? (((i >> 1) & 1) | (i & 4)) : (4 * ((i >> 1) & 1)))));
+        uint32_t o_zb = lds_addr(ldsZ);
+        asm volatile("; addresses of the loop" : "+v"(px_wr), "+v"(o_px_rd), "+v"(o_twA), "+v"(o_twB), "+v"(q_tr), "+v"(q_zr), "+v"(o_zb), "+v"(st_off) : : TIC_RSV_CLOBBER);
+        const uint8_t *px_rd = lds_ptr<const uint8_t>(o_px_rd);
+        uint32_t *twA = lds_ptr<uint32_t>(o_twA), *twB = lds_ptr<uint32_t>(o_twB);
+        const uint4 *tr = reinterpret_cast<const uint4 *>(__builtin_assume_aligned(ldsT, 16)) + q_tr;
+        const uint4 *zr = reinterpret_cast<const uint4 *>(__builtin_assume_aligned(ldsZ, 16)) + q_zr;
+        char *zb = lds_ptr<char>(o_zb);
+        out_f = reinterpret_cast<int16_t *>(reinterpret_cast<char *>(w.out) + (long)blockIdx.z * w.frame_stride_out);
         asm volatile("s_waitcnt vmcnt(2)\n\tv_mov_b32 %0, v76\n\tv_mov_b32 %1, v77\n\tv_mov_b32 %2, v78\n\tv_mov_b32 %3, v79"
                      : "=v"(c_fill.x), "=v"(c_fill.y), "=v"(c_fill.z), "=v"(c_fill.w) : : "memory", "v76", "v77", "v78", "v79");
         if (lane < kStripBlkPieces / kWavesPerWG) *reinterpret_cast<u32x4 *>(cst_blk + (wave * (kStripBlkPieces / kWavesPerWG) + lane) * 16) = c_fill;
@@ -449,12 +473,10 @@
         zzv = *reinterpret_cast<const u32x4 *>(cst_blk + (kCols ? kBlkZz : kBlkZzT) + i * 16);
         auto zz_ptr = [&](uint32_t ofs) {
             const uint32_t c = ofs >> 4;
-            return reinterpret_cast<int16_t *>(ldsZ + c * 128 + (ofs & 15) + 16 * (b ^ (kCols ? (((c >> 1) & 1) | (c & 4)) : (4 * ((c >> 1) & 1)))));
+            return reinterpret_cast<int16_t *>(zb + c * 128 + (ofs & 15) + 16 * (b ^ (kCols ? (((c >> 1) & 1) | (c & 4)) : (4 * ((c >> 1) & 1)))));
         };
         int16_t *zp0 = zz_ptr(zzv.x & 0xffff), *zp1 = zz_ptr(zzv.x >> 16), *zp2 = zz_ptr(zzv.y & 0xffff), *zp3 = zz_ptr(zzv.y >> 16);
         int16_t *zp4 = zz_ptr(zzv.z & 0xffff), *zp5 = zz_ptr(zzv.z >> 16), *zp6 = zz_ptr(zzv.w & 0xffff), *zp7 = zz_ptr(zzv.w >> 16);
-        const uint4 *zr = reinterpret_cast<const uint4 *>(
-            __builtin_assume_aligned(ldsZ + 16 * (i * 8 + (b ^ (kCols ? (((i >> 1) & 1) | (i & 4)) : (4 * ((i >> 1) & 1))))), 16));
         wave_lds_fence();
 
         int left = n_my;
@@ -516,7 +538,7 @@
             wave_lds_fence();
             const uint4 val = *zr;
             wave_lds_fence();
-            const char *dst = reinterpret_cast<const char *>(a.out) + ((unsigned long long)ob << 7);
+            const char *dst = reinterpret_cast<const char *>(out_f) + ((unsigned long long)ob << 7);
             const unsigned long long mG = cA | (cB & ~kRat);
             if (__builtin_expect(mG != 0ull, 0)) {
                 const uint32_t gm = (uint32_t)__ballot(((mG >> (8u * (uint32_t)i)) & 0xffull) != 0ull) & 0xffu;
@@ -563,10 +585,16 @@
 #undef TIC_STEP
         asm volatile("; end of the strip walk" : : : TIC_RSV_CLOBBER);
 #undef TIC_LOAD
+#undef TIC_LOAD_HEAD
 #undef TIC_TAKE_COLS
 #undef TIC_TAKE_ROWS
 #undef TIC_RSV_CLOBBER
     }
+    typedef const __attribute__((address_space(4))) char *kernarg_ptr;
+    kernarg_ptr kargs = (kernarg_ptr)__builtin_amdgcn_kernarg_segment_ptr();
+    asm volatile("; rare paths: DctqArgs from here on" : "+s"(kargs));
+    const __attribute__((address_space(4))) DctqArgs *ca = reinterpret_cast<const __attribute__((address_space(4))) DctqArgs *>(kargs + offsetof(StripKernargs, a));
+    (void)a;
     if (nE != 0) {
         const double *cst_cos = reinterpret_cast<const double *>(cst_blk + kBlkCos);
         const double *cst_rdiv = reinterpret_cast<const double *>(cst_blk + kBlkRdiv);
@@ -617,13 +645,13 @@
         }
         wave_lds_fence();
         const uint4 val = bat_img[e * 8 + i];
-        if (have) store16_wt_nt(reinterpret_cast<char *>(a.out) + ((unsigned long long)blk << 7) + (uint32_t)i * 16u, val);
-    }
-    if (a.fallback_count != nullptr && lane == 0) {
-        if (n_second != 0) atomicAdd(a.fallback_count, (unsigned long long)n_second);
-        if (n_quad != 0) atomicAdd(a.fallback_count + 1, (unsigned long long)n_quad);
-        if (mask_exact != 0ull) atomicAdd(a.fallback_count + 2, (unsigned long long)__builtin_popcountll(mask_exact));
-        if (nE != 0) atomicMax(a.fallback_count + 3, (unsigned long long)nE);
+        if (have) store16_wt_nt(reinterpret_cast<char *>(out_f) + ((unsigned long long)blk << 7) + (uint32_t)i * 16u, val);
+    }
+    if (ca->fallback_count != nullptr && lane == 0) {
+        if (n_second != 0) atomicAdd(ca->fallback_count, (unsigned long long)n_second);
+        if (n_quad != 0) atomicAdd(ca->fallback_count + 1, (unsigned long long)n_quad);
+        if (mask_exact != 0ull) atomicAdd(ca->fallback_count + 2, (unsigned long long)__builtin_popcountll(mask_exact));
+        if (nE != 0) atomicMax(ca->fallback_count + 3, (unsigned long long)nE);
     }
     if (mask_exact == 0ull) return;
     asm volatile("s_waitcnt vmcnt(0)" : : : "memory");
@@ -632,20 +660,20 @@
                             (uint16_t)zzn.z, (uint16_t)(zzn.z >> 16), (uint16_t)zzn.w, (uint16_t)(zzn.w >> 16)};
     for (unsigned long long todo = mask_exact; todo != 0ull; todo &= todo - 1ull) {
         const int k = __builtin_ctzll(todo);
-        const long t = (long)t_first + (long)k * a.tstep;
-        const int ty = (int)(t / a.fast_tx), tx = (int)(t - (long)ty * a.fast_tx);
+        const long t = (long)t_first + (long)k * ca->tstep;
+        const int ty = (int)(t / ca->fast_tx), tx = (int)(t - (long)ty * ca->fast_tx);
         Strip s;
         s.by = ty;
         s.bx = tx * 8 + b;
         s.valid = true;
-        s.oblk = (size_t)ty * a.bw + s.bx;
+        s.oblk = (size_t)ty * ca->bw + s.bx;
         uint32_t lo, hi;
-        load_block_row(a.img, a.h, a.w, a.stride, true, s, i, lo, hi);
+        load_block_row(img_s, ca->h, ca->w, ca->stride, true, s, i, lo, hi);
         transpose8x8_bytes(lo, hi, i);
         int q[8];
         const uint32_t und = second_level_8(lo, hi, ldsT, b, i, reinterpret_cast<const double *>(cst_blk + kBlkMul64), q);
         if (__ballot(und != 0u) != 0ull) exact_block(lo, hi, ldsT, b, i, C, q);
-        store_zigzag(reinterpret_cast<uint32_t *>(ldsZ), b, i, zz, q, a.out, s);
+        store_zigzag(reinterpret_cast<uint32_t *>(ldsZ), b, i, zz, q, out_f, s);
     }
 }
 
@@ -909,106 +937,43 @@
         }
     }
     const int bh = a.ntiles / a.tiles_x;
-    a.fast_tx = (a.aligned8 && (long)a.h * a.stride < (1L << 32)) ? a.w / 64 : 0;
-    a.fast_ty = a.h / 8;
-    const int nfast = a.fast_tx * a.fast_ty;
-    if (nfast > 0) {
-        const int max_strips = kMaxStripsPerWave2;
-        int wgs = grid_for(nfast);
-        static int cus = 256;
-        static const int resident = [] {
-            int dev = 0, per_cu = 0;
-            hipDeviceProp_t prop;
-            if (hipGetDevice(&dev) == hipSuccess && hipGetDeviceProperties(&prop, dev) == hipSuccess) cus = prop.multiProcessorCount;
-            if (hipOccupancyMaxActiveBlocksPerMultiprocessor(&per_cu, dctq_strip_kernel<true>, kWavesPerWG * 64, 0) != hipSuccess || per_cu < 1)
-                per_cu = 4;
-            if (per_cu > 6) per_cu = 6;
-            return cus * per_cu;
-        }();
-        const Tunables tune = tunables();
-        const int cap_env = tune.max_wgs > 0 ? tune.max_wgs : resident;
-        int cap = cap_env / nf;
-        if (cap < 64) cap = 64;
-        if (wgs > cap) wgs = cap;
-        const int min_wgs = (nfast + kWavesPerWG * max_strips - 1) / (kWavesPerWG * max_strips);
-        if (wgs < min_wgs) wgs = min_wgs;
-        a.nwaves = wgs * kWavesPerWG;
-        a.wg_stride = kWavesPerWG;
-        a.tstep = a.nwaves;
-        a.wg_span = nfast;
-        a.round_wgs = 0;
-        a.team_count = 0;
-        const int S = tune.chunk < 1 ? 1 : (tune.chunk > max_strips ? max_strips : tune.chunk);
-        const int min_wgs16 = (nfast + kWavesPerWG * kMaxStripsPerWave - 1) / (kWavesPerWG * kMaxStripsPerWave);
-        const bool multi_round = (long)min_wgs16 * nf > (long)cap_env;
-        if (tune.sched == 1 && multi_round) {
-            a.wg_stride = a.wg_span = kWavesPerWG * S;
-            a.tstep = kWavesPerWG;
-            wgs = (nfast + a.wg_stride - 1) / a.wg_stride;
-            a.nwaves = wgs * kWavesPerWG;
-        } else if (tune.sched == 2 && multi_round && nf == 1) {
-            a.round_wgs = cap_env;
-            a.wg_span = kWavesPerWG * S;
-            a.tstep = a.round_wgs * kWavesPerWG;
-            wgs = (nfast + a.wg_span - 1) / a.wg_span;
-            wgs = (wgs + a.round_wgs - 1) / a.round_wgs * a.round_wgs;
-            a.nwaves = wgs * kWavesPerWG;
-        }
-        if (!multi_round && nf == 1 && tune.split[0] > 0 && wgs == cap_env && wgs % cus == 0 && wgs / cus <= 8) {
-            const int R = wgs / cus;
-            a.team_count = cus;
-            a.tstep = cus * kWavesPerWG;
-            const int rows_total = (nfast + a.tstep - 1) / a.tstep;
-            double wsum = 0;
-            for (int r = 0; r < R; r++) wsum += tune.split[r] > 0 ? tune.split[r] : 1;
-            double acc = 0;
-            a.split[0] = 0;
-            for (int r = 0; r < R; r++) {
-                acc += tune.split[r] > 0 ? tune.split[r] : 1;
-                a.split[r + 1] = (int)(rows_total * acc / wsum + 0.5);
-                if (a.split[r + 1] - a.split[r] > max_strips) a.team_count = 0;
-            }
-            a.split[R] = rows_total;
-            if (rows_total > 255) a.team_count = 0;
-            if (a.team_count == 0) a.tstep = a.nwaves;
-        }
-        a.step_ty = a.tstep / a.fast_tx;
-        a.step_tx = a.tstep % a.fast_tx;
-        a.in_step32 = (uint32_t)((long)a.step_ty * 8 * a.stride + (long)a.step_tx * 64);
-        a.in_wrap32 = (uint32_t)(8 * a.stride - (long)a.fast_tx * 64);
-        a.oblk_step = (uint32_t)((long)a.step_ty * a.bw + (long)a.step_tx * 8);
-        a.oblk_wrap = (uint32_t)((long)a.bw - (long)a.fast_tx * 8);
-        dim3 grid(wgs, 1, nf);
-        const unsigned long long dmax = (unsigned long long)(a.round_wgs > 0 ? a.round_wgs : a.tstep);
-        if ((unsigned long long)nfast * (unsigned long long)a.fast_tx >= (1ull << 32) ||
-            ((unsigned long long)nfast + dmax) * dmax >= (1ull << 32)) {
-            a.fast_tx = a.fast_ty = 0;
-        } else {
-            auto magic = [](long d) { return d <= 1 ? 0u : (uint32_t)((1ull << 32) / (unsigned long long)d + 1ull); };
-            a.magic_fast_tx = magic(a.fast_tx);
-            a.magic_tstep = magic(a.round_wgs > 0 ? a.round_wgs : a.tstep);
-            a.split_lo = a.split_hi = 0;
-            if (a.team_count > 0) {
-                const int R = wgs / a.team_count;
-                for (int k = 0; k <= R; k++) {
-                    if (k < 8) a.split_lo |= (unsigned long long)(a.split[k] & 0xff) << (8 * k);
-                    else a.split_hi = (unsigned long long)(a.split[k] & 0xff);
-                }
-                grid = dim3(a.team_count, R, nf);
-            }
-            const bool cols = tune.order < 0 ? !multi_round : tune.order == 1;
-            if (ev_start && ev_stop) {
-                if (cols)
-                    hipExtLaunchKernelGGL(dctq_strip_kernel<true>, grid, block, 0, stream, ev_start, ev_stop, 0, a);
-                else
-                    hipExtLaunchKernelGGL(dctq_strip_kernel<false>, grid, block, 0, stream, ev_start, ev_stop, 0, a);
-            } else if (cols)
-                hipLaunchKernelGGL(dctq_strip_kernel<true>, grid, block, 0, stream, a);
-            else
-                hipLaunchKernelGGL(dctq_strip_kernel<false>, grid, block, 0, stream, a);
-        }
-    } else {
-        a.fast_tx = a.fast_ty = 0;
+    static int cus = 256;
+    static const int resident = [] {
+        int dev = 0, per_cu = 0;
+        hipDeviceProp_t prop;
+        if (hipGetDevice(&dev) == hipSuccess && hipGetDeviceProperties(&prop, dev) == hipSuccess) cus = prop.multiProcessorCount;
+        if (hipOccupancyMaxActiveBlocksPerMultiprocessor(&per_cu, dctq_strip_kernel<true>, kWavesPerWG * 64, 0) != hipSuccess || per_cu < 1)
+            per_cu = 4;
+        if (per_cu > 6) per_cu = 6;
+        return cus * per_cu;
+    }();
+    const Tunables tune = tunables();
+    StripTune st;
+    st.cus = cus, st.resident = resident, st.max_wgs = tune.max_wgs, st.sched = tune.sched, st.chunk = tune.chunk;
+    for (int k = 0; k < 8; k++) st.split[k] = tune.split[k];
+    const StripFrame fr = {a.h, a.w, a.stride, a.bw, a.aligned8, nf};
+    const StripPlan pl = strip_plan(fr, st);
+    a.fast_tx = pl.fast_tx;
+    a.fast_ty = pl.fast_ty;
+    if (pl.launch) {
+        a.nwaves = pl.nwaves, a.wg_stride = pl.wg_stride, a.tstep = pl.tstep, a.wg_span = pl.wg_span, a.round_wgs = pl.round_wgs;
+        a.team_count = pl.team_count, a.step_ty = pl.step_ty, a.step_tx = pl.step_tx;
+        for (int k = 0; k < 9; k++) a.split[k] = pl.split[k];
+        a.in_step32 = pl.hd.in_step32, a.in_wrap32 = pl.in_wrap32, a.oblk_step = pl.wm.oblk_step, a.oblk_wrap = pl.wm.oblk_wrap;
+        a.magic_fast_tx = pl.hd.magic_fast_tx, a.magic_tstep = pl.wm.magic_round_wgs;
+        a.split_lo = pl.hd.split, a.split_hi = (pl.hd.misc >> 8) & 0xffu;
+        const StripHead &hd = pl.hd;
+        StripWarm wm = pl.wm;
+        wm.out = a.out, wm.frame_stride_in = a.frame_stride_in, wm.frame_stride_out = a.frame_stride_out;
+        const dim3 grid(pl.grid_x, pl.grid_y, nf);
+        const bool cols = tune.order < 0 ? !pl.multi_round : tune.order == 1;
+        auto *kern = cols ? dctq_strip_kernel<true> : dctq_strip_kernel<false>;
+        if (ev_start && ev_stop)
+            hipExtLaunchKernelGGL(kern, grid, block, 0, stream, ev_start, ev_stop, 0, a.img, a.consts, hd.split, hd.stride, hd.misc, hd.tstep, hd.nfast,
+                                  hd.fast_tx, hd.magic_fast_tx, hd.in_step32, hd.step_tx, wm, a);
+        else
+            hipLaunchKernelGGL(kern, grid, block, 0, stream, a.img, a.consts, hd.split, hd.stride, hd.misc, hd.tstep, hd.nfast, hd.fast_tx,
+                               hd.magic_fast_tx, hd.in_step32, hd.step_tx, wm, a);
     }
     const int nrem = bh * (a.tiles_x - a.fast_tx) + (bh - a.fast_ty) * a.fast_tx;
     if (nrem > 0) {
diff --git a/tinyimgcodec_amd/csrc/tic_strip_plan.h b/tinyimgcodec_amd/csrc/tic_strip_plan.h
--- /dev/null
+++ b/tinyimgcodec_amd/csrc/tic_strip_plan.h
@@ -0,0 +1,227 @@
+#pragma once
+#include <stdint.h>
+
+#if defined(__HIPCC__) || defined(__CUDACC__)
+#define TIC_PLAN_HD __host__ __device__ __forceinline__
+#else
+#define TIC_PLAN_HD inline
+#endif
+
+namespace tic {
+
+constexpr int kStripWavesPerWG = 4;
+constexpr int kStripMaxPerWave = 64;
+constexpr int kStripResidentPerWave = 16;
+enum : uint32_t { kStripRows = 0, kStripChunk = 1, kStripRound = 2 };
+
+struct StripHead {
+    unsigned long long split;
+    uint32_t stride;
+    uint32_t misc;
+    uint32_t tstep;
+    uint32_t nfast;
+    uint32_t fast_tx;
+    uint32_t magic_fast_tx;
+    uint32_t in_step32;
+    uint32_t step_tx;
+};
+struct alignas(64) StripWarm {
+    int16_t *out;
+    long frame_stride_in, frame_stride_out;
+    uint32_t oblk_step, oblk_wrap;
+    uint32_t bw;
+    uint32_t round_wgs, round_span, magic_round_wgs;
+};
+static_assert(sizeof(StripWarm) == 64, "one cache line");
+
+struct StripCursor {
+    uint32_t t_first;
+    uint32_t txp;
+    uint32_t ty;
+    uint32_t in_off;
+    int n_my;
+};
+
+TIC_PLAN_HD uint32_t strip_mulhi(uint32_t a, uint32_t b) { return (uint32_t)(((unsigned long long)a * b) >> 32); }
+TIC_PLAN_HD uint32_t strip_in_wrap(const StripHead &h) { return 8u * h.stride - 64u * h.fast_tx; }
+
+TIC_PLAN_HD StripCursor strip_cursor(const StripHead &h, const StripWarm &w, uint32_t bx, uint32_t by, uint32_t wave) {
+    const uint32_t kind = h.misc & 0xffu;
+    uint32_t tf;
+    int n;
+    if (kind == kStripRows) {
+        const uint32_t row0 = (uint32_t)(h.split >> (8u * (by & 7u))) & 0xffu;
+        const uint32_t row1 = by < 7u ? (uint32_t)(h.split >> (8u * by + 8u)) & 0xffu : (h.misc >> 8) & 0xffu;
+        const uint32_t rows = row1 - row0;
+        tf = row0 * h.tstep + bx * (uint32_t)kStripWavesPerWG + wave;
+        const uint32_t last = tf + (rows - 1u) * h.tstep;
+        n = (int)rows - (last >= h.nfast ? 1 : 0);
+        n = n < 0 ? 0 : n;
+    } else if (kind == kStripChunk) {
+        const uint32_t span = ((h.misc >> 16) & 0xffu) * (uint32_t)kStripWavesPerWG;
+        const uint32_t base = bx * span;
+        const uint32_t lim = base + span < h.nfast ? base + span : h.nfast;
+        tf = base + wave;
+        n = tf < lim ? (int)((lim - tf + (uint32_t)kStripWavesPerWG - 1u) / (uint32_t)kStripWavesPerWG) : 0;
+    } else {
+        const uint32_t rho = w.magic_round_wgs ? strip_mulhi(bx, w.magic_round_wgs) : bx;
+        const uint32_t wl = bx - rho * w.round_wgs;
+        const uint32_t base = rho * w.round_wgs * w.round_span;
+        const uint32_t lim = base + w.round_wgs * w.round_span < h.nfast ? base + w.round_wgs * w.round_span : h.nfast;
+        tf = base + wl * (uint32_t)kStripWavesPerWG + wave;
+        n = tf < lim ? (int)((lim - tf + h.tstep - 1u) / h.tstep) : 0;
+    }
+    StripCursor c;
+    c.n_my = n;
+    c.t_first = n == 0 ? 0u : tf;
+    const uint32_t ty = h.magic_fast_tx ? strip_mulhi(c.t_first, h.magic_fast_tx) : c.t_first;
+    c.txp = c.t_first - ty * h.fast_tx;
+    c.ty = ty;
+    c.in_off = ty * (8u * h.stride) + c.txp * 64u;
+    return c;
+}
+TIC_PLAN_HD uint32_t strip_oblk(uint32_t ty, uint32_t txp, const StripWarm &w) { return ty * w.bw + txp * 8u; }
+
+TIC_PLAN_HD bool strip_step_in(uint32_t &txp, uint32_t &in_off, uint32_t step_tx, uint32_t fast_tx, uint32_t in_step32, uint32_t in_wrap32) {
+    txp += step_tx, in_off += in_step32;
+    const bool wrap = txp >= fast_tx;
+    if (__builtin_expect(wrap, 0)) txp -= fast_tx, in_off += in_wrap32;
+    return wrap;
+}
+TIC_PLAN_HD void strip_step_blk(uint32_t &oblk, bool wrap, const StripWarm &w) { oblk += w.oblk_step + (wrap ? w.oblk_wrap : 0u); }
+TIC_PLAN_HD void strip_step(uint32_t &txp, uint32_t &in_off, uint32_t &oblk, uint32_t step_tx, uint32_t fast_tx, uint32_t in_step32, uint32_t in_wrap32,
+                            const StripWarm &w) {
+    txp += step_tx, in_off += in_step32, oblk += w.oblk_step;
+    if (__builtin_expect(txp >= fast_tx, 0)) txp -= fast_tx, in_off += in_wrap32, oblk += w.oblk_wrap;
+}
+
+struct StripFrame {
+    int h, w;
+    long stride;
+    int bw;
+    int aligned8;
+    int nframes;
+};
+struct StripTune {
+    int cus, resident;
+    int max_wgs;
+    int sched;
+    int chunk;
+    int split[8];
+};
+struct StripPlan {
+    bool launch;
+    bool multi_round;
+    int fast_tx, fast_ty;
+    uint32_t grid_x, grid_y;
+    StripHead hd;
+    StripWarm wm;
+    int nwaves, wg_stride, tstep, wg_span, round_wgs, team_count, step_ty, step_tx;
+    int split[9];
+    uint32_t in_wrap32;
+};
+
+inline uint32_t strip_magic(long d) { return d <= 1 ? 0u : (uint32_t)((1ull << 32) / (unsigned long long)d + 1ull); }
+
+inline StripPlan strip_plan(const StripFrame &f, const StripTune &tune) {
+    StripPlan p{};
+    const int W = kStripWavesPerWG, max_strips = kStripMaxPerWave;
+    const int nf = f.nframes > 0 ? f.nframes : 1;
+    p.fast_tx = (f.aligned8 && (long)f.h * f.stride < (1L << 32)) ? f.w / 64 : 0;
+    p.fast_ty = f.h / 8;
+    const int nfast = p.fast_tx * p.fast_ty;
+    if (nfast <= 0) {
+        p.fast_tx = p.fast_ty = 0;
+        return p;
+    }
+    int wgs = (nfast + W - 1) / W;
+    const int cap_env = tune.max_wgs > 0 ? tune.max_wgs : tune.resident;
+    int cap = cap_env / nf;
+    if (cap < 64) cap = 64;
+    if (wgs > cap) wgs = cap;
+    const int min_wgs = (nfast + W * max_strips - 1) / (W * max_strips);
+    if (wgs < min_wgs) wgs = min_wgs;
+    p.nwaves = wgs * W;
+    p.wg_stride = W;
+    p.tstep = p.nwaves;
+    p.wg_span = nfast;
+    uint32_t kind = kStripRows;
+    const int S = tune.chunk < 1 ? 1 : (tune.chunk > max_strips ? max_strips : tune.chunk);
+    const int min_wgs16 = (nfast + W * kStripResidentPerWave - 1) / (W * kStripResidentPerWave);
+    p.multi_round = (long)min_wgs16 * nf > (long)cap_env;
+    if (tune.sched == 1 && p.multi_round) {
+        kind = kStripChunk;
+        p.wg_stride = p.wg_span = W * S;
+        p.tstep = W;
+        wgs = (nfast + p.wg_stride - 1) / p.wg_stride;
+        p.nwaves = wgs * W;
+    } else if (tune.sched == 2 && p.multi_round && nf == 1) {
+        kind = kStripRound;
+        p.round_wgs = cap_env;
+        p.wg_span = W * S;
+        p.tstep = p.round_wgs * W;
+        wgs = (nfast + p.wg_span - 1) / p.wg_span;
+        wgs = (wgs + p.round_wgs - 1) / p.round_wgs * p.round_wgs;
+        p.nwaves = wgs * W;
+    }
+    p.grid_x = (uint32_t)wgs, p.grid_y = 1;
+    int R = 1;
+    if (kind == kStripRows) {
+        p.split[0] = 0;
+        p.split[1] = (nfast + p.tstep - 1) / p.tstep;
+    }
+    if (!p.multi_round && nf == 1 && tune.split[0] > 0 && wgs == cap_env && tune.cus > 0 && wgs % tune.cus == 0 && wgs / tune.cus <= 8) {
+        const int Rt = wgs / tune.cus;
+        const int tstep = tune.cus * W;
+        const int rows_total = (nfast + tstep - 1) / tstep;
+        int split[9] = {0};
+        bool ok = rows_total <= 255;
+        double wsum = 0, acc = 0;
+        for (int r = 0; r < Rt; r++) wsum += tune.split[r] > 0 ? tune.split[r] : 1;
+        for (int r = 0; r < Rt; r++) {
+            acc += tune.split[r] > 0 ? tune.split[r] : 1;
+            split[r + 1] = r + 1 == Rt ? rows_total : (int)(rows_total * acc / wsum + 0.5);
+        }
+        for (int r = 0; r < Rt; r++)
+            if (split[r + 1] - split[r] > max_strips) ok = false;
+        if (ok) {
+            p.team_count = tune.cus;
+            p.tstep = tstep;
+            R = Rt;
+            for (int r = 0; r <= Rt; r++) p.split[r] = split[r];
+            p.grid_x = (uint32_t)tune.cus, p.grid_y = (uint32_t)Rt;
+        }
+    }
+    p.step_ty = p.tstep / p.fast_tx;
+    p.step_tx = p.tstep % p.fast_tx;
+    const unsigned long long dmax = (unsigned long long)(p.round_wgs > 0 ? p.round_wgs : p.tstep);
+    if ((unsigned long long)nfast * (unsigned long long)p.fast_tx >= (1ull << 32) || ((unsigned long long)nfast + dmax) * dmax >= (1ull << 32)) {
+        p.fast_tx = p.fast_ty = 0;
+        return p;
+    }
+    p.launch = true;
+    StripHead &h = p.hd;
+    h.split = 0;
+    h.misc = kind | ((uint32_t)(kind == kStripChunk ? S : 0) << 16);
+    if (kind == kStripRows)
+        for (int k = 0; k <= R; k++) {
+            if (k < 8) h.split |= (unsigned long long)(p.split[k] & 0xff) << (8 * k);
+            else h.misc |= (uint32_t)(p.split[k] & 0xff) << 8;
+        }
+    h.stride = (uint32_t)f.stride;
+    h.tstep = (uint32_t)p.tstep;
+    h.nfast = (uint32_t)nfast;
+    h.fast_tx = (uint32_t)p.fast_tx;
+    h.magic_fast_tx = strip_magic(p.fast_tx);
+    h.in_step32 = (uint32_t)((long)p.step_ty * 8 * f.stride + (long)p.step_tx * 64);
+    h.step_tx = (uint32_t)p.step_tx;
+    p.in_wrap32 = strip_in_wrap(h);
+    p.wm.oblk_step = (uint32_t)((long)p.step_ty * f.bw + (long)p.step_tx * 8);
+    p.wm.oblk_wrap = (uint32_t)((long)f.bw - (long)p.fast_tx * 8);
+    p.wm.bw = (uint32_t)f.bw;
+    p.wm.round_wgs = (uint32_t)p.round_wgs;
+    p.wm.round_span = (uint32_t)(kind == kStripRound ? p.wg_span : 0);
+    p.wm.magic_round_wgs = kind == kStripRound ? strip_magic(p.round_wgs) : 0u;
+    return p;
+}
+}
```
